# yangfei1223/CRFConv

Hardware: AMD Instinct MI355X
Metric: M points/sec fwd+bwd, S3DIS 40960-pt cloud, K=16, 3 CRF iters; mIoU parity (higher is better)
Workload: dtype f32; 1 GPU; BASELINE configs[1]: S3DIS-like synthetic clouds (one point per 4 cm voxel of an 8x8x3 m box), 4 clouds x 40960 pts per GPU, K=16, ratios [4,4,4,4,2], PointConvBig(in=6, classes=13, use_crf, steps=3), train mode: fwd + weighted CE + bwd + flat-bucket grad all-reduce + SGD(momentum) step; tables resident in HBM; point order from the device collate: morton; global_batch=4, points_per_cloud=40960, parallelism=dp1 (batch-sharded)

## Files before the change

### crfconv_amd/_lib.py

```python
import ctypes
import os

_HERE = os.path.dirname(os.path.abspath(__file__))
LIB_PATH = os.environ.get('CRFCONV_LIB') or os.path.join(_HERE, 'libcrfconv_amd.so')

_vp, _i, _i64, _sz, _f = ctypes.c_void_p, ctypes.c_int, ctypes.c_int64, ctypes.c_size_t, ctypes.c_float
_d = ctypes.c_double
_u64 = ctypes.c_uint64

SIGNATURES = {
    'crfconv_abi_version': (_i, []),
    'crfconv_last_error': (ctypes.c_char_p, []),
    'crfconv_knn': (_i, [_vp, _sz, _sz, _vp, _sz, _sz, _vp]),
    'crfconv_knn_omp': (_i, [_vp, _sz, _sz, _vp, _sz, _sz, _vp]),
    'crfconv_knn_batch': (_i, [_vp, _sz, _sz, _sz, _vp, _sz, _sz, _vp]),
    'crfconv_knn_batch_omp': (_i, [_vp, _sz, _sz, _sz, _vp, _sz, _sz, _vp]),
    'crfconv_knn_batch_dev_workspace': (_sz, [_sz, _sz, _sz, _sz]),
    'crfconv_knn_batch_dev': (_i, [_vp, _sz, _sz, _sz, _vp, _sz, _sz, _vp, _vp, _vp, _sz, _vp]),
    'crfconv_fps': (_i, [_vp, _i, _vp, _vp, _vp, _vp, _vp, _vp, _vp, _vp]),
    'crfconv_grid_subsample': (_i64, [_vp, _i64, _vp, _i, _vp, _i, _f, _vp, _vp, _vp, _i64]),
    'crfconv_grid_subsample_dev_workspace': (_sz, [_i64, _i, _i]),
    'crfconv_grid_subsample_dev': (_i64, [_vp, _i64, _vp, _i, _vp, _i, _f, _vp, _vp, _vp, _i64, _vp, _sz, _vp]),
    'crfconv_index_narrow': (_i, [_vp, _i64, _i64, _i, _i64, _vp, _vp, _vp, _vp]),
    'crfconv_index_narrow_sorted': (_i, [_vp, _i64, _i64, _i, _i64, _i, _vp, _vp, _vp, _vp]),
# ... 18 lines not shown
    'crfconv_wide_bwd_edge': (_i, [_vp, _vp, _vp, _i, _i, _i64, _i, _vp, _i, _vp]),
    'crfconv_wide_scatter': (_i, [_vp, _vp, _vp, _vp, _i, _i64, _i, _vp, _i, _vp, _vp]),
    'crfconv_wide_similarity_bwd': (_i, [_vp, _vp, _vp, _vp, _i, _i, _i64, _i, _vp, _vp, _vp]),
    'crfconv_similarity_bwd': (_i, [_vp, _vp, _vp, _vp, _i, _i, _i64, _i, _vp, _vp, _vp]),
    'crfconv_similarity_bwd_scatter': (_i, [_vp, _vp, _vp, _vp, _vp, _i, _i, _i64, _i, _vp, _vp]),
    'crfconv_pointconv_workspace': (_sz, [_i64, _i, _i]),
    'crfconv_pointconv_moments_packed': (_i, [_vp, _vp, _vp, _i, _i64, ctypes.c_double, _vp, _vp, _vp, _vp, _vp, _sz, _vp]),
    'crfconv_pointconv_moments': (_i, [_vp, _vp, _vp, _i, _i64, _vp, _vp, _sz, _vp]),
    'crfconv_pointconv_stats': (_i, [_vp, _vp, _vp, _i, _i64, _i, _vp, _vp, _vp, _f, _vp, _vp, _vp, _vp, _sz, _vp]),
    'crfconv_pointconv_forward_uv': (_i, [_vp, _vp, _vp, _vp, _i, _i64, _i, _vp, _vp, _vp, _f, _vp, _vp, _vp, _vp, _vp, _vp, _sz, _vp, _vp]),
    'crfconv_pointconv_forward_uv_hosts': (_i, [_i, _i]),
    'crfconv_pointconv_forward_uv_hosting': (_i, [_vp, _vp, _vp, _vp, _i, _i64, _i, _vp, _vp, _vp, _f, _vp, _vp, _vp, _vp, _vp, _vp, _sz, _vp,
                                                  _vp, _vp, _i, _vp, _vp, _vp]),
    'crfconv_pointconv_combine': (_i, [_vp, _vp, _vp, _vp, _vp, _vp, _d, _vp, _vp, _f, _f, _i64, _i, _vp, _vp, _vp, _vp, _vp]),
    'crfconv_pointconv_bwd_reduce_uv': (_i, [_vp, _vp, _vp, _i64, _i, _vp, _vp, _vp, _d, _i, _vp, _vp, _vp, _vp, _vp, _vp, _sz, _vp, _vp]),
    'crfconv_pointconv_forward': (_i, [_vp, _vp, _vp, _vp, _i, _i64, _i, _vp, _vp, _vp, _f, _vp, _vp, _vp, _vp]),
    'crfconv_pointconv_bwd_reduce': (_i, [_vp, _vp, _vp, _vp, _vp, _i, _i64, _i, _vp, _vp, _vp, _f, _vp, _vp, _vp, _sz, _vp]),
    'crfconv_pointconv_bwd_params': (_i, [_vp, _vp, _vp, _vp, _vp, _i, _i64, _i, _vp, _vp, _vp, _f, _vp, _vp, _vp,
                                          _vp, _vp, _vp, _sz, _vp]),
    'crfconv_pointconv_bwd_dump': (_i, [_vp, _vp, _vp, _vp, _vp, _i, _i64, _i, _vp, _vp, _vp, _f, _vp, _vp, _vp, _vp, _vp, _vp, _vp]),
    'crfconv_pointconv_bwd_a1_workspace': (_sz, [_i64, _i]),
    'crfconv_pointconv_bwd_a1': (_i, [_vp, _vp, _vp, _i64, _i, _f, _vp, _vp, _sz, _vp]),
    'crfconv_pointconv_bwd_input': (_i, [_vp, _vp, _vp, _vp, _vp, _i, _i64, _i, _vp, _vp, _vp, _f, _vp, _vp, _vp, _vp]),
    'crfconv_pointconv_bwd_input_reduce': (_i, [_vp, _vp, _vp, _vp, _vp, _i, _i64, _i64, _i, _vp, _vp, _vp, _f, _vp, _vp, _vp, _vp, _vp, _vp, _vp, _vp, _d, _i,
                                                _vp, _vp, _vp, _vp, _vp, _vp, _sz, _vp, _vp]),
    'crfconv_pointconv_fold1': (_i, [_vp, _vp, _vp, _vp, ctypes.c_double, _vp, _vp, _f, _f, _i, _i, _vp, _vp, _vp, _vp]),
    'crfconv_pointconv_fold1_batched': (_i, [_vp, _i, _vp]),
    'crfconv_pointconv_fold1_bwd_batched': (_i, [_vp, _i, _vp]),
    'crfconv_pointconv_fold1_bwd': (_i, [_vp, _vp, _vp, _vp, _vp, _f, _i, _i, _vp, _vp, _vp, _vp, _vp, _vp]),
    'crfconv_pointconv_fold2': (_i, [_vp, _vp, _vp, _vp, ctypes.c_double, _vp, _vp, _f, _f, _i, _i, _vp, _vp, _vp, _vp]),
    'crfconv_pointconv_fold2_bwd': (_i, [_vp, _vp, _vp, _vp, ctypes.c_double, _i, _i, _vp, _vp, _vp, _vp, _vp, _vp]),
    'crfconv_linear_wgrad_workspace': (_sz, [_i64, _i, _i]),
    'crfconv_linear_wgrad': (_i, [_vp, _vp, _i64, _i, _i, _vp, _vp, _vp, _sz, _vp]),
    'crfconv_random_subsets': (_i, [_vp, _vp, _vp, _vp, _i, _u64, _vp, _vp]),
    'crfconv_upindex_workspace': (_sz, [_i64, _i64]),
    'crfconv_upindex_from_table': (_i, [_vp, _vp, _vp, _vp, _i64, _i64, _i, _i64, _vp, _vp, _sz, _vp]),
    'crfconv_gather_rows_batched': (_i, [_vp, _vp, _vp, _i, _vp, _i, _i64, _i64, _i64, _vp]),
    'crfconv_argsort_codes_workspace': (_sz, [_i64, _i64]),
    'crfconv_argsort_codes': (_i, [_vp, _i64, _i64, _vp, _vp, _sz, _vp]),
    'crfconv_gridsync_workspace': (_sz, []),
    'crfconv_gridsync_fail_word': (_i, []),
    'crfconv_mlp_small_supported': (_i, [_i64, _i, _i]),
    'crfconv_mlp_small_workspace': (_sz, [_i64, _i]),
    'crfconv_mlp_small_forward': (_i, [_vp, _vp, _i64, _i, _i, _vp, _vp, _vp, _vp, _f, _f, _f, _vp, _vp, _vp, _vp, _sz, _vp, _sz, _vp]),
    'crfconv_mlp_small_forward_join': (_i, [_vp, _vp, _i64, _i, _i, _vp, _vp, _vp, _vp, _f, _f, _f, _vp, _f, _vp, _vp, _vp, _vp, _sz, _vp, _sz, _vp]),
    'crfconv_ticket_bytes': (_sz, []),
    'crfconv_mlp_backward_supported': (_i, [_i64, _i, _i]),
    'crfconv_mlp_backward_workspace': (_sz, [_i64, _i, _i]),
    'crfconv_mlp_backward': (_i, [_vp, _vp, _vp, _vp, _vp, _f, _i64, _i, _i, _vp, _vp, _vp, _vp, _vp, _sz, _vp, _vp]),
    'crfconv_linear_forward_cat': (_i, [_vp, _vp, _i, _vp, _vp, _i64, _i, _i, _vp, _vp, _vp]),
    'crfconv_linear_forward_uv_supported': (_i, [_i, _i]),
    'crfconv_linear_forward_uv': (_i, [_vp, _vp, _i64, _i, _i, _vp, _vp, _vp]),
    'crfconv_mlp_small_forward_uv_supported': (_i, [_i]),
    'crfconv_mlp_small_forward_join_uv': (_i, [_vp, _vp, _i64, _i, _i, _vp, _vp, _vp, _vp, _f, _f, _f, _vp, _f, _vp, _vp, _vp, _vp, _sz, _vp, _sz, _vp]),
    'crfconv_gemm_stats_uv_supported': (_i, [_i64, _i, _i]),
    'crfconv_gemm_stats_uv': (_i, [_vp, _vp, _i64, _i, _i, _vp, _vp, _vp]),
    'crfconv_mlp_dw_jobs': (_i, [_vp, _i, _vp]),
    'crfconv_mlp_dw_jobs_hosting': (_i, [_vp, _i, _vp, _vp, _vp, _vp, _vp, _i, _vp, _vp]),
    'crfconv_mlp_backward_add': (_i, [_vp, _vp, _vp, _vp, _vp, _f, _i64, _i, _i, _vp, _vp, _vp, _vp, _vp, _vp, _sz, _vp, _vp]),
    'crfconv_mlp_backward_add_mask': (_i, [_vp, _vp, _vp, _vp, _vp, _f, _i64, _i, _i, _vp, _f, _vp, _vp, _vp, _vp, _vp, _sz, _vp, _vp]),
    'crfconv_mlp_backward_cat': (_i, [_vp, _vp, _vp, _vp, _i, _vp, _vp, _f, _i64, _i, _i, _vp, _vp, _vp, _vp, _vp, _vp, _sz, _vp, _vp]),
    'crfconv_bn_workspace': (_sz, [_i64, _i]),
    'crfconv_bn_forward': (_i, [_vp, _i64, _i, _vp, _vp, _vp, _vp, _f, _f, _i, _f, _vp, _vp, _vp, _sz, _vp]),
    'crfconv_bn_backward': (_i, [_vp, _vp, _vp, _i64, _i, _i, _f, _vp, _vp, _vp, _vp, _sz, _vp]),
    'crfconv_bn_apply': (_i, [_vp, _i64, _i, _vp, _f, _vp, _vp]),
    'crfconv_pointconv_bwd_params_slabs': (_i, [_vp, _i64, _i, _vp, _vp, _vp]),
    'crfconv_pointconv_bwd_a1_nblk': (_i64, [_i64, _i]),
    'crfconv_reduce_jobs_f64': (_i, [_vp, _i, _vp]),
    'crfconv_pointconv_bwd_dump_jobs': (_i, [_vp, _i, _vp]),
    'crfconv_pointconv_bwd_a1_jobs': (_i, [_vp, _i, _vp]),
    'crfconv_pointconv_wide_params_supported': (_i, [_i64, _i, _i]),
    'crfconv_pointconv_wide_params_nblk': (_i64, [_i64, _i]),
    'crfconv_pointconv_wide_params_jobs': (_i, [_vp, _i, _vp]),
    'crfconv_gemm_jobs': (_i, [_vp, _i, _vp]),
    'crfconv_linear_wgrad_nblk': (_i, [_i64, _i, _i]),
    'crfconv_linear_wgrad_partial_jobs': (_i, [_vp, _i, _vp]),
    'crfconv_linear_wgrad_partial': (_i, [_vp, _vp, _i64, _i, _i, _i, _vp, _sz, _vp, _vp]),
    'crfconv_morton_codes': (_i, [_vp, _i64, _i64, _vp, _vp, _vp]),
    'crfconv_copy_jobs': (_i, [_vp, _i, _vp]),
    'crfconv_index_narrow_batched': (_i, [_vp, _i, _vp]),
    'crfconv_pointconv_moments_batched_workspace': (_sz, [_vp, _i]),
    'crfconv_pointconv_moments_batched': (_i, [_vp, _i, _vp, _sz, _vp]),
    'crfconv_reduce_jobs_both': (_i, [_vp, _i, _vp, _i, _vp]),
    'crfconv_reduce_jobs': (_i, [_vp, _i, _vp]),
    'crfconv_linear_forward_supported': (_i, [_i, _i]),
    'crfconv_linear_forward_stat_records': (_sz, [_i64]),
# ... 111 lines not shown
    _fields_ = [('x', ctypes.c_void_p), ('gout', ctypes.c_void_p), ('pos_src', ctypes.c_void_p), ('pos_tgt', ctypes.c_void_p),
                ('idx32', ctypes.c_void_p), ('K', ctypes.c_int32), ('m_tgt', ctypes.c_int64), ('d', ctypes.c_int32), ('A1', ctypes.c_void_p),
                ('b1', ctypes.c_void_p), ('W2', ctypes.c_void_p), ('slope', ctypes.c_float), ('ca', ctypes.c_void_p), ('cb', ctypes.c_void_p),
                ('cc', ctypes.c_void_p), ('dw2_partial', ctypes.c_void_p), ('a1_partial', ctypes.c_void_p)]


class PcA1Job(ctypes.Structure):
    _fields_ = [('gw', ctypes.c_void_p), ('h1', ctypes.c_void_p), ('rel', ctypes.c_void_p), ('n_edges', ctypes.c_int64), ('d', ctypes.c_int32),
                ('slope', ctypes.c_float), ('workspace', ctypes.c_void_p), ('workspace_bytes', ctypes.c_size_t)]


class GemmJob(ctypes.Structure):
    _fields_ = [('A', ctypes.c_void_p), ('B', ctypes.c_void_p), ('C', ctypes.c_void_p), ('M', ctypes.c_int64), ('N', ctypes.c_int32),
                ('K', ctypes.c_int32)]


class GemmStatsJob(ctypes.Structure):
    _fields_ = [('A', ctypes.c_void_p), ('B', ctypes.c_void_p), ('M', ctypes.c_int64), ('N', ctypes.c_int32), ('K', ctypes.c_int32),
                ('C', ctypes.c_void_p), ('stat_rec', ctypes.c_void_p)]


class BnApplyJob(ctypes.Structure):
    _fields_ = [('stat_rec', ctypes.c_void_p), ('nrec', ctypes.c_int64), ('x', ctypes.c_void_p), ('M', ctypes.c_int64), ('C', ctypes.c_int32),
                ('gamma', ctypes.c_void_p), ('beta', ctypes.c_void_p), ('run_mean', ctypes.c_void_p), ('run_var', ctypes.c_void_p),
                ('momentum', ctypes.c_float), ('eps', ctypes.c_float), ('skip', ctypes.c_void_p), ('slope', ctypes.c_float),
                ('coef', ctypes.c_void_p), ('y', ctypes.c_void_p)]


class MlpBwdJob(ctypes.Structure):
    _fields_ = [('gA', ctypes.c_void_p), ('Y', ctypes.c_void_p), ('coef', ctypes.c_void_p), ('W', ctypes.c_void_p), ('addend', ctypes.c_void_p),
                ('M', ctypes.c_int64), ('Ci', ctypes.c_int32), ('Co', ctypes.c_int32), ('training', ctypes.c_int32), ('slope', ctypes.c_float),
                ('gY', ctypes.c_void_p), ('dX', ctypes.c_void_p), ('dgamma', ctypes.c_void_p), ('dbeta', ctypes.c_void_p),
                ('workspace', ctypes.c_void_p), ('workspace_bytes', ctypes.c_size_t),
                ('mask_ref', ctypes.c_void_p), ('mask_slope', ctypes.c_float)]


class UvFold(ctypes.Structure):
    _fields_ = [('U', ctypes.c_void_p), ('V', ctypes.c_void_p), ('stats', ctypes.c_void_p), ('shift', ctypes.c_void_p),
                ('gamma2', ctypes.c_void_p), ('beta2', ctypes.c_void_p), ('n_edges', ctypes.c_double), ('run_mean', ctypes.c_void_p),
                ('run_var', ctypes.c_void_p), ('momentum', ctypes.c_float), ('eps', ctypes.c_float), ('a2', ctypes.c_void_p),
                ('b2', ctypes.c_void_p), ('aux2', ctypes.c_void_p), ('out', ctypes.c_void_p)]


class Reduce64Job(ctypes.Structure):
    _fields_ = [('partial', ctypes.c_void_p), ('is_float', ctypes.c_int32), ('nblk', ctypes.c_int64), ('nslots', ctypes.c_int32),
                ('out', ctypes.c_void_p)]


class WgradJob(ctypes.Structure):
    _fields_ = [('G', ctypes.c_void_p), ('X', ctypes.c_void_p), ('M', ctypes.c_int64), ('Co', ctypes.c_int32), ('Ci', ctypes.c_int32),
                ('want_bias', ctypes.c_int32), ('workspace', ctypes.c_void_p), ('workspace_bytes', ctypes.c_size_t)]


class RevJob(ctypes.Structure):
    _fields_ = [('idx32', ctypes.c_void_p), ('E', ctypes.c_int64), ('m_src', ctypes.c_int64), ('rev_ptr', ctypes.c_void_p),
                ('rev_eid', ctypes.c_void_p)]


class NarrowJob(ctypes.Structure):
    _fields_ = [('idx64', ctypes.c_void_p), ('B', ctypes.c_int64), ('n_tgt', ctypes.c_int64), ('K', ctypes.c_int32),
                ('n_src', ctypes.c_int64), ('sort_from', ctypes.c_int32), ('idx32', ctypes.c_void_p), ('idx16', ctypes.c_void_p),
                ('bad_count', ctypes.c_void_p)]


class MomentsJob(ctypes.Structure):
    _fields_ = [('pos_src', ctypes.c_void_p), ('pos_tgt', ctypes.c_void_p), ('idx32', ctypes.c_void_p), ('K', ctypes.c_int32),
                ('m_tgt', ctypes.c_int64), ('n_edges', ctypes.c_double), ('mean', ctypes.c_void_p), ('cov', ctypes.c_void_p),
                ('packed', ctypes.c_void_p), ('mean32', ctypes.c_void_p)]


class Fold1Job(ctypes.Structure):
    _fields_ = [('W1', ctypes.c_void_p), ('gamma1', ctypes.c_void_p), ('beta1', ctypes.c_void_p), ('mom', ctypes.c_void_p),
                ('n_edges', ctypes.c_double), ('run_mean', ctypes.c_void_p), ('run_var', ctypes.c_void_p),
                ('momentum', ctypes.c_float), ('eps', ctypes.c_float), ('use_batch', ctypes.c_int32), ('d', ctypes.c_int32),
                ('A1', ctypes.c_void_p), ('b1', ctypes.c_void_p), ('aux1', ctypes.c_void_p)]


class Fold1BwdJob(ctypes.Structure):
    _fields_ = [('W1', ctypes.c_void_p), ('gamma1', ctypes.c_void_p), ('mom', ctypes.c_void_p), ('aux1', ctypes.c_void_p),
                ('dA1b1', ctypes.c_void_p), ('eps', ctypes.c_float), ('use_batch', ctypes.c_int32), ('d', ctypes.c_int32),
                ('pad_', ctypes.c_int32), ('dW1', ctypes.c_void_p), ('dgamma1', ctypes.c_void_p), ('dbeta1', ctypes.c_void_p),
                ('dW2_f64', ctypes.c_void_p), ('dW2_f32', ctypes.c_void_p)]


# ... 47 lines not shown
```

### crfconv_amd/csrc/gemm.hip

```cpp
#include "common.hpp"
#include "gridsync.hpp"
#include "uv_fold.hpp"

#include <cstdlib>

namespace crf {

using gf32x4 = __attribute__((ext_vector_type(4))) float;

#ifndef GM_BK_
#define GM_BK_ 32
#endif
#ifndef GM_PF_
#define GM_PF_ 2
#endif
#ifndef GM_WAIT_SLEEP_
#define GM_WAIT_SLEEP_ 4
#endif
constexpr int GM_BLOCK = 256, GM_BK = GM_BK_;
constexpr int GM_PF = GM_PF_;
static_assert(GM_PF >= 2 && GM_PF % 2 == 0, "an even number of register sets (the LDS buffers alternate)");

template <bool VEC>
__device__ __forceinline__ float4 gm_ld4(const float* __restrict__ p, int valid) {
    float4 v = make_float4(0.f, 0.f, 0.f, 0.f);
    if constexpr (VEC) {
        if (valid > 0) v = *reinterpret_cast<const float4*>(p);
    } else {
        if (valid > 0) v.x = p[0];
        if (valid > 1) v.y = p[1];
        if (valid > 2) v.z = p[2];
        if (valid > 3) v.w = p[3];
    }
    return v;
}

constexpr int GM_PRO_MAXK = 512;
struct GemmPro {
    const float* Y;
    const float* coef;
    const float* fin;
    float slope;
    float* gY;
    unsigned* sync = nullptr;
    unsigned need = 0, nprod = 0;
    unsigned* fail = nullptr;
    const float* mref = nullptr;
    float mslope = 1.f;
};
constexpr int GM_PRO_LDS = 6 * GM_PRO_MAXK + 4;

template <int WM, int WN, int WR, int WC, bool BNK, bool PRO>
constexpr int gemm_lds_floats() {
    constexpr int BM = 16 * WM * WR, BN = 16 * WN * WC;
    return (PRO ? GM_PRO_LDS : 0) + 2 * BM * (GM_BK + 4) + 2 * (BNK ? BN * (GM_BK + 4) : GM_BK * (BN + 4));
}

constexpr int GM_UV_MAXK = 128;
template <int WM, int WN, int WR, int WC, bool BNK, bool VEC, bool PRO, bool STATS, bool UV = false>
__device__ __forceinline__ void gemm_tile(const float* __restrict__ A, const float* __restrict__ B,
                                          const float* __restrict__ bias, const float* __restrict__ addend,
                                          int M, int N, int K, float* __restrict__ C, const GemmPro& pro,
                                          float* __restrict__ stat_rec, const unsigned bx, const unsigned by,
                                          float* __restrict__ lds ,
                                          const unsigned gridx = 0 ,
                                          const UvFold* __restrict__ uv = nullptr, float* __restrict__ uvc = nullptr) {
    static_assert(WR * WC * WAVE == GM_BLOCK, "four wavefronts");
    static_assert(!UV || (VEC && !PRO), "the combine prologue: aligned widths, not the dX product");
    static_assert(!PRO || (VEC && !BNK), "the prologue form is the dX product of aligned widths");
    constexpr int BM = 16 * WM * WR, BN = 16 * WN * WC;
    constexpr int LDA = GM_BK + 4;
    constexpr int LDN = GM_BK + 4;
    constexpr int LDK = BN + 4;
    constexpr int TA = BM * LDA, TB = BNK ? BN * LDN : GM_BK * LDK;
    constexpr int NA4 = BM * GM_BK / 4, NB4 = BN * GM_BK / 4;
    constexpr int PA = (NA4 + GM_BLOCK - 1) / GM_BLOCK, PB = (NB4 + GM_BLOCK - 1) / GM_BLOCK;
    float* const sPro = lds;
    float (*sA)[TA] = reinterpret_cast<float (*)[TA]>(lds + (PRO ? GM_PRO_LDS : 0));
    float (*sB)[TB] = reinterpret_cast<float (*)[TB]>(lds + (PRO ? GM_PRO_LDS : 0) + 2 * TA);
    const int lane = threadIdx.x & 63, wave = threadIdx.x >> 6;
    const int rr = lane & 15, g = lane >> 4;
    const int wr = wave / WC, wc = wave - wr * WC;
    const int m0 = bx * BM, n0 = by * BN;
    const float4 zero4 = make_float4(0.f, 0.f, 0.f, 0.f);

    struct Regs { float4 a[PA], b[PB], y[(PRO || UV) ? PA : 1]; int kc; };
    auto fetch = [&](int kc, Regs& r) {
        r.kc = kc;
#pragma unroll
        for (int i = 0; i < PA; ++i) {
            const int q = threadIdx.x + GM_BLOCK * i;
            r.a[i] = zero4;
            if constexpr (PRO || UV) r.y[i] = zero4;
            if (NA4 % GM_BLOCK != 0 && q >= NA4) continue;
            const int row = m0 + q / (GM_BK / 4), k = kc + 4 * (q % (GM_BK / 4));
            if (row < M) r.a[i] = gm_ld4<VEC>(A + (int64_t)row * K + k, K - k);
            if constexpr (PRO) {
                if (row < M) r.y[i] = gm_ld4<VEC>(pro.Y + (int64_t)row * K + k, K - k);
            }
            if constexpr (UV) {
                if (row < M) r.y[i] = gm_ld4<VEC>(uv->V + (int64_t)row * K + k, K - k);
            }
        }
#pragma unroll
        for (int i = 0; i < PB; ++i) {
            const int q = threadIdx.x + GM_BLOCK * i;
            r.b[i] = zero4;
            if (NB4 % GM_BLOCK != 0 && q >= NB4) continue;
            if constexpr (BNK) {
                const int n = n0 + q / (GM_BK / 4), k = kc + 4 * (q % (GM_BK / 4));
                if (n < N) r.b[i] = gm_ld4<VEC>(B + (int64_t)n * K + k, K - k);
            } else {
                const int k = kc + q / (BN / 4), n = n0 + 4 * (q % (BN / 4));
                if (k < K) r.b[i] = gm_ld4<VEC>(B + (int64_t)k * N + n, N - n);
            }
        }
    };
    auto park = [&](int buf, const Regs& r) {
#pragma unroll
        for (int i = 0; i < PA; ++i) {
            const int q = threadIdx.x + GM_BLOCK * i;
            if (NA4 % GM_BLOCK != 0 && q >= NA4) continue;
            float4 av = r.a[i];
            if constexpr (PRO) {
                const int row = m0 + q / (GM_BK / 4), k = r.kc + 4 * (q % (GM_BK / 4));
                if (row < M && k < K) {
                    const float4 ca = *reinterpret_cast<const float4*>(sPro + k), cb = *reinterpret_cast<const float4*>(sPro + GM_PRO_MAXK + k);
                    const float4 mu = *reinterpret_cast<const float4*>(sPro + 2 * GM_PRO_MAXK + k), rs = *reinterpret_cast<const float4*>(sPro + 3 * GM_PRO_MAXK + k);
                    const float4 c2 = *reinterpret_cast<const float4*>(sPro + 4 * GM_PRO_MAXK + k), c3 = *reinterpret_cast<const float4*>(sPro + 5 * GM_PRO_MAXK + k);
// ... 160 lines not shown
                    s2[e] += __shfl_xor(s2[e], o, WAVE);
                }
            }
            if (rr == 0 && n < N) {
#pragma unroll
                for (int e = 0; e < 4; ++e)
                    *reinterpret_cast<float4*>(stat_rec + ((int64_t)rec * N + n + e) * 4) = make_float4(sv[e], (float)nrows, s1[e], s2[e]);
            }
        }
    }
#pragma unroll
    for (int i = 0; i < WM; ++i) {
        const int row = m0 + 16 * (wr * WM + i) + rr;
        if (row >= M) continue;
#pragma unroll
        for (int j = 0; j < WN; ++j) {
            const int n = n0 + 16 * (wc * WN + j) + 4 * g;
            if (n >= N) continue;
            float4 o = make_float4(acc[i][j][0], acc[i][j][1], acc[i][j][2], acc[i][j][3]);
            if (addend != nullptr) {
                const float4 a4 = gm_ld4<VEC>(addend + (int64_t)row * N + n, N - n);
                o.x += a4.x; o.y += a4.y; o.z += a4.z; o.w += a4.w;
            }
            if constexpr (PRO) {
                if (pro.mref != nullptr) {
                    const float4 r4 = gm_ld4<VEC>(pro.mref + (int64_t)row * N + n, N - n);
                    o.x = r4.x > 0.f ? o.x : pro.mslope * o.x;
                    o.y = r4.y > 0.f ? o.y : pro.mslope * o.y;
                    o.z = r4.z > 0.f ? o.z : pro.mslope * o.z;
                    o.w = r4.w > 0.f ? o.w : pro.mslope * o.w;
                }
            }
            float* cp = C + (int64_t)row * N + n;
            if constexpr (VEC) {
                *reinterpret_cast<float4*>(cp) = o;
            } else {
                cp[0] = o.x;
                if (n + 1 < N) cp[1] = o.y;
                if (n + 2 < N) cp[2] = o.z;
                if (n + 3 < N) cp[3] = o.w;
            }
        }
    }
    if constexpr (PRO) {
        if (pro.sync != nullptr && threadIdx.x == 0) {
            const unsigned local = bx + by * gridx, g = local % (unsigned)WL_GROUPS;
            const unsigned n_in_group = pro.nprod / WL_GROUPS + (g < pro.nprod % WL_GROUPS ? 1u : 0u);
            unsigned* gt = pro.sync + (WL_REPL + g) * FW_LINE;
            if (__hip_atomic_fetch_add(gt, 1u, __ATOMIC_RELAXED, __HIP_MEMORY_SCOPE_AGENT) + 1 == n_in_group) {
                __hip_atomic_store(gt, 0u, __ATOMIC_RELAXED, __HIP_MEMORY_SCOPE_AGENT);
                unsigned* top = pro.sync + (WL_REPL + WL_GROUPS) * FW_LINE;
                const unsigned groups = pro.nprod < (unsigned)WL_GROUPS ? pro.nprod : (unsigned)WL_GROUPS;
                if (__hip_atomic_fetch_add(top, 1u, __ATOMIC_RELAXED, __HIP_MEMORY_SCOPE_AGENT) + 1 == groups) {
                    __hip_atomic_store(top, 0u, __ATOMIC_RELAXED, __HIP_MEMORY_SCOPE_AGENT);
                    for (int r = 0; r < WL_REPL; ++r) __hip_atomic_store(pro.sync + r * FW_LINE, 0u, __ATOMIC_RELAXED, __HIP_MEMORY_SCOPE_AGENT);
                }
            }
        }
    }
}

template <int WM, int WN, int WR, int WC, bool BNK, bool VEC, bool PRO = false, bool STATS = false>
__global__ __launch_bounds__(GM_BLOCK) void gemm_kernel(const float* __restrict__ A, const float* __restrict__ B,
                                                        const float* __restrict__ bias, const float* __restrict__ addend,
                                                        int M, int N, int K, float* __restrict__ C, const GemmPro pro = GemmPro(),
                                                        float* __restrict__ stat_rec = nullptr) {
// ... 27 lines not shown
static inline bool gm_wide(int64_t M, int N) { return N >= GM_WIDE_MIN_N_ && ((M + 31) / 32) * (int64_t)((N + 31) / 32) >= GM_WIDE_MIN_TILES_; }
struct GemmStatsJobs {
    const float* A[GG_MAX]; const float* B[GG_MAX]; float* C[GG_MAX]; float* rec[GG_MAX];
    int M[GG_MAX], N[GG_MAX], K[GG_MAX], tiles_x[GG_MAX], wide[GG_MAX];
    int tile_base[GG_MAX + 1];
    int njobs;
};
__global__ __launch_bounds__(GM_BLOCK) void gemm_stats_jobs_kernel(const GemmStatsJobs t) {
    int j = 0;
    while (j + 1 < t.njobs && t.tile_base[j + 1] <= (int)blockIdx.x) ++j;
    const unsigned local = blockIdx.x - (unsigned)t.tile_base[j];
    const unsigned tx = (unsigned)uni(t.tiles_x[j]);
    const unsigned bx = (unsigned)uni((int)(local % tx)), by = (unsigned)uni((int)(local / tx));
    __shared__ __attribute__((aligned(16))) float lds[gemm_lds_floats<1, 2, 2, 2, true, false>()];
    if (uni(t.wide[j]))
        gemm_tile<1, 2, 2, 2, true, true, false, true>(uni(t.A[j]), uni(t.B[j]), nullptr, nullptr, uni(t.M[j]), uni(t.N[j]), uni(t.K[j]), uni(t.C[j]), GemmPro(),
                                                       uni(t.rec[j]), bx, by, lds);
    else
        gemm_tile<1, 1, 2, 2, true, true, false, true>(uni(t.A[j]), uni(t.B[j]), nullptr, nullptr, uni(t.M[j]), uni(t.N[j]), uni(t.K[j]), uni(t.C[j]), GemmPro(),
                                                       uni(t.rec[j]), bx, by, lds);
}
__global__ __launch_bounds__(GM_BLOCK) void gemm_stats_uv_kernel(const float* __restrict__ U, const float* __restrict__ B, const int M, const int N,
                                                                 const int K, float* __restrict__ C, float* __restrict__ rec, const int tiles_x,
                                                                 const int wide, const UvFold uv) {
    const unsigned tx = (unsigned)tiles_x;
    const unsigned bx = (unsigned)uni((int)(blockIdx.x % tx)), by = (unsigned)uni((int)(blockIdx.x / tx));
    __shared__ __attribute__((aligned(16))) float lds[gemm_lds_floats<1, 2, 2, 2, true, false>()];
    __shared__ __attribute__((aligned(16))) float s_uv[2 * GM_UV_MAXK];
    if (wide)
        gemm_tile<1, 2, 2, 2, true, true, false, true, true>(U, B, nullptr, nullptr, M, N, K, C, GemmPro(), rec, bx, by, lds, 0, &uv, s_uv);
    else
        gemm_tile<1, 1, 2, 2, true, true, false, true, true>(U, B, nullptr, nullptr, M, N, K, C, GemmPro(), rec, bx, by, lds, 0, &uv, s_uv);
}
struct GemmProJobs {
    const float* A[GG_MAX]; const float* B[GG_MAX]; const float* addend[GG_MAX]; float* C[GG_MAX];
    GemmPro pro[GG_MAX];
    int M[GG_MAX], N[GG_MAX], K[GG_MAX], tiles_x[GG_MAX], wide[GG_MAX];
    int tile_base[GG_MAX + 1];
    int njobs;
};
__global__ __launch_bounds__(GM_BLOCK) void gemm_pro_jobs_kernel(const GemmProJobs t) {
    int j = 0;
    while (j + 1 < t.njobs && t.tile_base[j + 1] <= (int)blockIdx.x) ++j;
    const unsigned local = blockIdx.x - (unsigned)t.tile_base[j];
    GemmPro pro;
    pro.Y = uni(t.pro[j].Y); pro.coef = uni(t.pro[j].coef); pro.fin = uni(t.pro[j].fin); pro.slope = uni(t.pro[j].slope); pro.gY = uni(t.pro[j].gY);
    pro.mref = uni(t.pro[j].mref); pro.mslope = uni(t.pro[j].mslope);
    const unsigned tx = (unsigned)uni(t.tiles_x[j]);
    const unsigned bx = (unsigned)uni((int)(local % tx)), by = (unsigned)uni((int)(local / tx));
    __shared__ __attribute__((aligned(16))) float lds[gemm_lds_floats<1, 2, 2, 2, false, true>()];
    if (uni(t.wide[j]))
        gemm_tile<1, 2, 2, 2, false, true, true, false>(uni(t.A[j]), uni(t.B[j]), nullptr, uni(t.addend[j]), uni(t.M[j]), uni(t.N[j]), uni(t.K[j]), uni(t.C[j]),
                                                        pro, nullptr, bx, by, lds, tx);
    else
        gemm_tile<1, 1, 2, 2, false, true, true, false>(uni(t.A[j]), uni(t.B[j]), nullptr, uni(t.addend[j]), uni(t.M[j]), uni(t.N[j]), uni(t.K[j]), uni(t.C[j]),
                                                        pro, nullptr, bx, by, lds, tx);
}

}

namespace crf {

constexpr int BT_ROWS = 128, BT_CH = 64, BT_NR = BT_ROWS / 16;
struct TileSumFin {
    unsigned* ticket;
    int ntile;
    int training;
    float inv_m;
    float* fin;
    float* dgamma;
    float* dbeta;
    unsigned* done = nullptr;
};
struct TileSumLds { float red[16][2][64]; int last; };
typedef unsigned int bt_u32x2 __attribute__((ext_vector_type(2)));
__device__ __forceinline__ void bn_bwd_tile_sums_body(const float* __restrict__ gA, const float* __restrict__ Y,
                                                       const float* __restrict__ coef, int M, int K, int tile_rows,
                                                       float slope, double* __restrict__ partial, const int bx, const int by,
                                                       const TileSumFin f, TileSumLds& L) {
    float (&s_red)[16][2][64] = L.red;
    int& s_last = L.last;
    const int cq = threadIdx.x & 15, rl = threadIdx.x >> 4;
    const int c = by * BT_CH + 4 * cq;
    const int row0 = bx * tile_rows;
    const int row_end = row0 + tile_rows < M ? row0 + tile_rows : M;
    float4 s1 = make_float4(0.f, 0.f, 0.f, 0.f), s2 = s1;
    if (c < K) {
        const float4 ca = *reinterpret_cast<const float4*>(coef + c), cb = *reinterpret_cast<const float4*>(coef + K + c);
// ... 70 lines not shown
        if (threadIdx.x < WL_REPL) __hip_atomic_fetch_add(f.done + threadIdx.x * FW_LINE, 1u, __ATOMIC_RELAXED, __HIP_MEMORY_SCOPE_AGENT);
    }
}

struct TileSumJobs {
    const float* gA[GG_MAX]; const float* Y[GG_MAX]; const float* coef[GG_MAX]; double* partial[GG_MAX];
    float* fin[GG_MAX]; float* dgamma[GG_MAX]; float* dbeta[GG_MAX];
    int M[GG_MAX], K[GG_MAX], tile_rows[GG_MAX], ntile[GG_MAX], training[GG_MAX];
    float slope[GG_MAX], inv_m[GG_MAX];
    unsigned* ticket;
    int blk_base[GG_MAX + 1];
    int njobs;
};
constexpr int BT_SLABS = GM_PRO_MAXK / BT_CH;
__device__ __forceinline__ void bn_bwd_tile_sums_job(const TileSumJobs& t, const int blk, TileSumLds& L, unsigned* const* done = nullptr) {
    int j = 0;
    while (j + 1 < t.njobs && t.blk_base[j + 1] <= blk) ++j;
    const int local = blk - t.blk_base[j];
    const int ntile = uni(t.ntile[j]);
    const int bx = local % ntile, by = local / ntile;
    TileSumFin f;
    f.ticket = uni(t.ticket) + (j * BT_SLABS + by) * FW_LINE; f.ntile = ntile; f.training = uni(t.training[j]); f.inv_m = uni(t.inv_m[j]);
    f.fin = uni(t.fin[j]); f.dgamma = uni(t.dgamma[j]); f.dbeta = uni(t.dbeta[j]);
    f.done = done != nullptr ? uni(done[j]) : nullptr;
    bn_bwd_tile_sums_body(uni(t.gA[j]), uni(t.Y[j]), uni(t.coef[j]), uni(t.M[j]), uni(t.K[j]), uni(t.tile_rows[j]), uni(t.slope[j]), uni(t.partial[j]),
                          bx, by, f, L);
}
__global__ __launch_bounds__(256) void bn_bwd_tile_sums_jobs_kernel(const TileSumJobs t) {
    __shared__ TileSumLds L;
    bn_bwd_tile_sums_job(t, (int)blockIdx.x, L);
}

struct SmallBwdSync { unsigned* done[GG_MAX]; int nsum; };
__global__ __launch_bounds__(GM_BLOCK) void mlp_small_bwd_jobs_kernel(const TileSumJobs ts, const GemmProJobs t, const SmallBwdSync sy) {
    __shared__ __attribute__((aligned(16))) float lds[gemm_lds_floats<1, 2, 2, 2, false, true>()];
    static_assert(sizeof(TileSumLds) <= sizeof(lds), "the tile-sum workgroups use the product's buffer");
    if ((int)blockIdx.x < sy.nsum) {
        bn_bwd_tile_sums_job(ts, (int)blockIdx.x, *reinterpret_cast<TileSumLds*>(lds), sy.done);
        return;
    }
    const int blk = (int)blockIdx.x - sy.nsum;
    int j = 0;
    while (j + 1 < t.njobs && t.tile_base[j + 1] <= blk) ++j;
    const unsigned local = (unsigned)(blk - t.tile_base[j]);
    GemmPro pro;
    pro.Y = uni(t.pro[j].Y); pro.coef = uni(t.pro[j].coef); pro.fin = uni(t.pro[j].fin); pro.slope = uni(t.pro[j].slope); pro.gY = uni(t.pro[j].gY);
    pro.mref = uni(t.pro[j].mref); pro.mslope = uni(t.pro[j].mslope);
    pro.sync = uni(t.pro[j].sync); pro.need = (unsigned)uni((int)t.pro[j].need); pro.nprod = (unsigned)uni((int)t.pro[j].nprod); pro.fail = uni(t.pro[j].fail);
    const unsigned tx = (unsigned)uni(t.tiles_x[j]);
    const unsigned bx = (unsigned)uni((int)(local % tx)), by = (unsigned)uni((int)(local / tx));
    if (uni(t.wide[j]))
        gemm_tile<1, 2, 2, 2, false, true, true, false>(uni(t.A[j]), uni(t.B[j]), nullptr, uni(t.addend[j]), uni(t.M[j]), uni(t.N[j]), uni(t.K[j]), uni(t.C[j]),
                                                        pro, nullptr, bx, by, lds, tx);
    else
        gemm_tile<1, 1, 2, 2, false, true, true, false>(uni(t.A[j]), uni(t.B[j]), nullptr, uni(t.addend[j]), uni(t.M[j]), uni(t.N[j]), uni(t.K[j]), uni(t.C[j]),
                                                        pro, nullptr, bx, by, lds, tx);
}
}

extern "C" int crfconv_mlp_small_backward_supported(int64_t M, int Ci, int Co) {
    return (M >= 1 && M < (int64_t)1 << 24 && Ci >= 4 && Co >= 4 && Ci % 4 == 0 && Co % 4 == 0 && Co <= crf::GM_PRO_MAXK) ? 1 : 0;
}

static void bt_plan(int64_t M, int& ntile, int& tile_rows) {
    constexpr int BT_MAXTILES = 48;
    int64_t rows = crf::BT_ROWS;
    if ((M + rows - 1) / rows > BT_MAXTILES) rows = (((M + BT_MAXTILES - 1) / BT_MAXTILES + 15) / 16) * 16;
    tile_rows = (int)rows;
    ntile = (int)((M + rows - 1) / rows);
}

static size_t bt_fin_offset(int Co, int ntile) { return (sizeof(double) * 2 * (size_t)Co * (size_t)ntile + 255) & ~(size_t)255; }
extern "C" size_t crfconv_mlp_small_backward_workspace(int64_t M, int Co) {
    if (M < 1 || Co < 1) return 0;
    int ntile, tile_rows;
    bt_plan(M, ntile, tile_rows);
    return bt_fin_offset(Co, ntile) + sizeof(float) * 2 * (size_t)Co + 512;
}

extern "C" int crfconv_mlp_small_backward(const float* gA, const float* Y, const float* coef, const float* W, const float* addend,
                                          int64_t M, int Ci, int Co, int training, float slope, float* gY, float* dX, float* dgamma,
                                          float* dbeta, void* workspace, size_t workspace_bytes, unsigned* ticket, void* stream) {
    crf_mlp_bwd_job job;
    job.gA = gA; job.Y = Y; job.coef = coef; job.W = W; job.addend = addend; job.M = M; job.Ci = Ci; job.Co = Co; job.training = training;
    job.slope = slope; job.gY = gY; job.dX = dX; job.dgamma = dgamma; job.dbeta = dbeta; job.workspace = workspace; job.workspace_bytes = workspace_bytes;
    job.mask_ref = nullptr; job.mask_slope = 1.f;
    return crfconv_mlp_small_backward_jobs(&job, 1, ticket, stream);
}

static int mlp_small_backward_jobs_impl(const crf_mlp_bwd_job* jobs, int njobs, unsigned* ticket, unsigned* sync_ws, void* stream);
extern "C" int crfconv_mlp_small_backward_jobs(const crf_mlp_bwd_job* jobs, int njobs, unsigned* ticket, void* stream) {
    return mlp_small_backward_jobs_impl(jobs, njobs, ticket, nullptr, stream);
}
extern "C" int crfconv_mlp_small_backward_jobs_one_launch(const crf_mlp_bwd_job* jobs, int njobs, unsigned* ticket, unsigned* sync_ws, void* stream) {
    CRF_REQUIRE(sync_ws != nullptr, CRF_ERR_ARG, "null barrier workspace");
    return mlp_small_backward_jobs_impl(jobs, njobs, ticket, sync_ws, stream);
}
static int mlp_small_backward_jobs_impl(const crf_mlp_bwd_job* jobs, int njobs, unsigned* ticket, unsigned* sync_ws, void* stream) {
    CRF_REQUIRE(jobs && ticket && njobs >= 1 && njobs <= crf::GG_MAX, CRF_ERR_ARG, "1 .. %d jobs (got %d) and the ticket words", crf::GG_MAX, njobs);
    crf::TileSumJobs ts;
    crf::GemmProJobs gp;
    crf::SmallBwdSync sy;
    for (int j = 0; j < crf::GG_MAX; ++j) sy.done[j] = nullptr;
    sy.nsum = 0;
    int64_t blocks = 0, tiles = 0;
    for (int j = 0; j <= crf::GG_MAX; ++j) {
        ts.blk_base[j] = (int)blocks;
        gp.tile_base[j] = (int)tiles;
        if (j >= crf::GG_MAX) break;
        if (j >= njobs) {
            ts.gA[j] = nullptr; ts.Y[j] = nullptr; ts.coef[j] = nullptr; ts.partial[j] = nullptr; ts.M[j] = 0; ts.K[j] = 4; ts.tile_rows[j] = crf::BT_ROWS;
            ts.ntile[j] = 1; ts.slope[j] = 1.f; ts.fin[j] = nullptr; ts.dgamma[j] = nullptr; ts.dbeta[j] = nullptr; ts.training[j] = 0; ts.inv_m[j] = 0.f;
            gp.A[j] = nullptr; gp.B[j] = nullptr; gp.addend[j] = nullptr; gp.C[j] = nullptr; gp.pro[j] = crf::GemmPro(); gp.M[j] = 0; gp.N[j] = 4; gp.K[j] = 4;
            gp.tiles_x[j] = 1; gp.wide[j] = 0;
            continue;
        }
        const crf_mlp_bwd_job& b = jobs[j];
        CRF_REQUIRE(b.gA && b.Y && b.coef && b.W && b.gY && b.dX && b.dgamma && b.dbeta && b.workspace, CRF_ERR_ARG, "job %d: null pointer", j);
        CRF_REQUIRE(crfconv_mlp_small_backward_supported(b.M, b.Ci, b.Co), CRF_ERR_UNSUPPORTED,
                    "job %d: mlp_small_backward %lld x %d -> %d: widths must be multiples of 4, Co <= %d", j, (long long)b.M, b.Ci, b.Co, crf::GM_PRO_MAXK);
        CRF_REQUIRE(b.workspace_bytes >= crfconv_mlp_small_backward_workspace(b.M, b.Co), CRF_ERR_WORKSPACE, "job %d: workspace too small", j);
        double* partial = reinterpret_cast<double*>((reinterpret_cast<uintptr_t>(b.workspace) + 255) & ~(uintptr_t)255);
        int ntile, tile_rows;
        bt_plan(b.M, ntile, tile_rows);
        ts.gA[j] = b.gA; ts.Y[j] = b.Y; ts.coef[j] = b.coef; ts.partial[j] = partial; ts.M[j] = (int)b.M; ts.K[j] = b.Co; ts.tile_rows[j] = tile_rows;
        float* fin = reinterpret_cast<float*>(reinterpret_cast<char*>(partial) + bt_fin_offset(b.Co, ntile));
        ts.ntile[j] = ntile; ts.slope[j] = b.slope; ts.fin[j] = fin; ts.dgamma[j] = b.dgamma; ts.dbeta[j] = b.dbeta; ts.training[j] = b.training;
        ts.inv_m[j] = (float)(1.0 / (double)b.M);
        blocks += (int64_t)ntile * ((b.Co + crf::BT_CH - 1) / crf::BT_CH);
        crf::GemmPro pro;
        pro.Y = b.Y; pro.coef = b.coef; pro.fin = fin; pro.slope = b.slope; pro.gY = b.gY;
        pro.mref = b.mask_ref; pro.mslope = b.mask_slope;
        gp.A[j] = b.gA; gp.B[j] = b.W; gp.addend[j] = b.addend; gp.C[j] = b.dX; gp.pro[j] = pro; gp.M[j] = (int)b.M; gp.N[j] = b.Ci; gp.K[j] = b.Co;
        gp.tiles_x[j] = (int)((b.M + 31) / 32);
        gp.wide[j] = crf::gm_wide(b.M, b.Ci) ? 1 : 0;
        const int64_t jt = (int64_t)gp.tiles_x[j] * ((b.Ci + (gp.wide[j] ? 63 : 31)) / (gp.wide[j] ? 64 : 32));
        tiles += jt;
        CRF_REQUIRE(tiles + blocks < ((int64_t)1 << 31), CRF_ERR_UNSUPPORTED, "too many tiles in one batch");
        if (sync_ws != nullptr) {
            gp.pro[j].sync = sync_ws + (crf::FW_WAIT + j * crf::WL_LINES) * crf::FW_LINE;
            gp.pro[j].need = (unsigned)((b.Co + crf::BT_CH - 1) / crf::BT_CH);
            gp.pro[j].nprod = (unsigned)jt;
            gp.pro[j].fail = sync_ws + crf::FW_FAIL * crf::FW_LINE;
            sy.done[j] = gp.pro[j].sync;
        }
    }
    ts.njobs = njobs;
    ts.ticket = ticket;
    gp.njobs = njobs;
    hipStream_t st = crf::as_stream(stream);
    if (sync_ws != nullptr) {
        sy.nsum = (int)blocks;
        hipLaunchKernelGGL(crf::mlp_small_bwd_jobs_kernel, dim3((unsigned)(blocks + tiles)), dim3(crf::GM_BLOCK), 0, st, ts, gp, sy);
        CRF_LAUNCH_CHECK();
        return CRF_OK;
    }
    hipLaunchKernelGGL(crf::bn_bwd_tile_sums_jobs_kernel, dim3((unsigned)blocks), dim3(256), 0, st, ts);
    CRF_LAUNCH_CHECK();
    hipLaunchKernelGGL(crf::gemm_pro_jobs_kernel, dim3((unsigned)tiles), dim3(crf::GM_BLOCK), 0, st, gp);
    CRF_LAUNCH_CHECK();
    return CRF_OK;
}

extern "C" size_t crfconv_gemm_stat_records(int64_t M) { return M < 1 ? 0 : (size_t)(2 * ((M + 31) / 32)); }

extern "C" int crfconv_gemm_stats(const float* A, const float* B, int64_t M, int N, int K, float* C, float* stat_rec, void* stream) {
    crf_gemm_stats_job job;
    job.A = A; job.B = B; job.M = M; job.N = N; job.K = K; job.C = C; job.stat_rec = stat_rec;
    return crfconv_gemm_stats_jobs(&job, 1, stream);
}

extern "C" int crfconv_gemm_stats_jobs(const crf_gemm_stats_job* jobs, int njobs, void* stream) {
    CRF_REQUIRE(jobs && njobs >= 1 && njobs <= crf::GG_MAX, CRF_ERR_ARG, "1 .. %d jobs (got %d)", crf::GG_MAX, njobs);
    crf::GemmStatsJobs t;
    int64_t tiles = 0;
    for (int j = 0; j <= crf::GG_MAX; ++j) {
        t.tile_base[j] = (int)tiles;
        if (j >= crf::GG_MAX) break;
        if (j >= njobs) {
            t.A[j] = nullptr; t.B[j] = nullptr; t.C[j] = nullptr; t.rec[j] = nullptr; t.M[j] = 0; t.N[j] = 4; t.K[j] = 4; t.tiles_x[j] = 1; t.wide[j] = 0;
            continue;
        }
        const crf_gemm_stats_job& b = jobs[j];
        CRF_REQUIRE(b.A && b.B && b.C && b.stat_rec, CRF_ERR_ARG, "job %d: null pointer", j);
        CRF_REQUIRE(b.M >= 1 && b.M < ((int64_t)1 << 31) && b.N >= 4 && b.K >= 4 && b.N % 4 == 0 && b.K % 4 == 0, CRF_ERR_UNSUPPORTED,
                    "job %d: gemm_stats %lld x %d x %d: N and K must be multiples of 4", j, (long long)b.M, b.N, b.K);
        t.A[j] = b.A; t.B[j] = b.B; t.C[j] = b.C; t.rec[j] = b.stat_rec; t.M[j] = (int)b.M; t.N[j] = b.N; t.K[j] = b.K;
        t.tiles_x[j] = (int)((b.M + 31) / 32);
        t.wide[j] = crf::gm_wide(b.M, b.N) ? 1 : 0;
        tiles += (int64_t)t.tiles_x[j] * ((b.N + (t.wide[j] ? 63 : 31)) / (t.wide[j] ? 64 : 32));
        CRF_REQUIRE(tiles < ((int64_t)1 << 31), CRF_ERR_UNSUPPORTED, "too many tiles in one batch");
    }
    t.njobs = njobs;
    hipLaunchKernelGGL(crf::gemm_stats_jobs_kernel, dim3((unsigned)tiles), dim3(crf::GM_BLOCK), 0, crf::as_stream(stream), t);
    CRF_LAUNCH_CHECK();
    return CRF_OK;
}

extern "C" int crfconv_gemm_stats_uv_supported(int64_t M, int N, int K) {
    return (M >= 1 && M < ((int64_t)1 << 31) && N >= 4 && K >= 4 && N % 4 == 0 && K % 4 == 0 && K <= crf::GM_UV_MAXK) ? 1 : 0;
}
extern "C" int crfconv_gemm_stats_uv(const crf_uv_fold* f, const float* B, int64_t M, int N, int K, float* C, float* stat_rec, void* stream) {
    CRF_REQUIRE(B && C && stat_rec, CRF_ERR_ARG, "null pointer");
    CRF_REQUIRE(crf::uv_fold_complete(f), CRF_ERR_ARG, "combine record: null pointer, or running statistics not as a pair");
    CRF_REQUIRE(crfconv_gemm_stats_uv_supported(M, N, K), CRF_ERR_UNSUPPORTED, "gemm_stats_uv %lld x %d x %d: N, K multiples of 4, K <= %d",
                (long long)M, N, K, crf::GM_UV_MAXK);
    const crf::UvFold uv = crf::uv_fold_args(f);
    const int tiles_x = (int)((M + 31) / 32), wide = crf::gm_wide(M, N) ? 1 : 0;
    const int64_t tiles = (int64_t)tiles_x * ((N + (wide ? 63 : 31)) / (wide ? 64 : 32));
    CRF_REQUIRE(tiles < ((int64_t)1 << 31), CRF_ERR_UNSUPPORTED, "too many tiles");
    hipLaunchKernelGGL(crf::gemm_stats_uv_kernel, dim3((unsigned)tiles), dim3(crf::GM_BLOCK), 0, crf::as_stream(stream), f->U, B, (int)M, N, K, C,
                       stat_rec, tiles_x, wide, uv);
    CRF_LAUNCH_CHECK();
    return CRF_OK;
}

extern "C" int crfconv_gemm_jobs(const crf_gemm_job* jobs, int njobs, void* stream) {
    CRF_REQUIRE(jobs || njobs == 0, CRF_ERR_ARG, "null pointer");
    CRF_REQUIRE(njobs >= 0, CRF_ERR_ARG, "njobs=%d < 0", njobs);
    hipStream_t st = crf::as_stream(stream);
    for (int j0 = 0; j0 < njobs; j0 += crf::GJ_MAX) {
        crf::GemmJobs t;
        const int n = njobs - j0 < crf::GJ_MAX ? njobs - j0 : crf::GJ_MAX;
        int64_t tiles = 0;
        for (int j = 0; j <= crf::GJ_MAX; ++j) {
            t.tile_base[j] = (int)tiles;
            if (j < n) {
                const crf_gemm_job& jb = jobs[j0 + j];
                CRF_REQUIRE(jb.A && jb.B && jb.C, CRF_ERR_ARG, "job %d: null pointer", j0 + j);
                CRF_REQUIRE(jb.M >= 1 && jb.M < ((int64_t)1 << 31) && jb.N >= 4 && jb.K >= 4 && jb.N % 4 == 0 && jb.K % 4 == 0, CRF_ERR_UNSUPPORTED,
                            "job %d: %lld x %d x %d (N, K multiples of 4)", j0 + j, (long long)jb.M, jb.N, jb.K);
                t.A[j] = jb.A; t.B[j] = jb.B; t.C[j] = jb.C; t.M[j] = (int)jb.M; t.N[j] = jb.N; t.K[j] = jb.K;
                t.tiles_x[j] = (int)((jb.M + 31) / 32);
                tiles += (int64_t)t.tiles_x[j] * ((jb.N + 31) / 32);
                CRF_REQUIRE(tiles < ((int64_t)1 << 31), CRF_ERR_UNSUPPORTED, "too many tiles in one batch");
            } else if (j < crf::GJ_MAX) {
                t.A[j] = nullptr; t.B[j] = nullptr; t.C[j] = nullptr; t.M[j] = 0; t.N[j] = 4; t.K[j] = 4; t.tiles_x[j] = 1;
            }
        }
        t.njobs = n;
        hipLaunchKernelGGL(crf::gemm_jobs_kernel, dim3((unsigned)tiles), dim3(crf::GM_BLOCK), 0, st, t);
        CRF_LAUNCH_CHECK();
    }
    return CRF_OK;
}
// ... 38 lines not shown
```

### crfconv_amd/csrc/linear.hip

```cpp
#include "common.hpp"
#include "gridsync.hpp"
#include "wgrad_body.hpp"
#include "crf_matrices_body.hpp"
#include "reduce64_body.hpp"
#include "uv_fold.hpp"

#include <cstdlib>

namespace crf {

template <int TCO, int TCI>
__global__ __launch_bounds__(WG_BLOCK) void wgrad_kernel(const float* __restrict__ G,
                                                         const float* __restrict__ X, int64_t M, int Co,
                                                         int Ci, int rows_per_block,
                                                         float* __restrict__ partial ,
                                                         float* __restrict__ partial_b ) {
    __shared__ float s_red[WG_RED_BUFS * TCO * TCI * 256];
    __shared__ float s_b[WG_WAVES * TCO * 16];
    wgrad_body<TCO, TCI>(G, X, M, Co, Ci, rows_per_block, partial, partial_b, blockIdx.x, blockIdx.y, blockIdx.z, s_red, s_b);
}

__global__ __launch_bounds__(WG_BLOCK) void wgrad_jobs_any_kernel(const WgJobTable t) {
    __shared__ float s_red[WG_RED_BUFS * 4 * 4 * 256];
    __shared__ float s_b[WG_WAVES * 4 * 16];
    wgrad_any_run(t, (int)blockIdx.x, s_red, s_b);
}


__device__ __forceinline__ void mlp_channel_part(int c, double s1, double s2, const float* __restrict__ coef, int64_t M, int Co,
                                                 float* __restrict__ dgamma, float* __restrict__ dbeta, float* __restrict__ bcoef) {
    dbeta[c] = (float)s1;
    dgamma[c] = (float)s2;
    const double a = coef[c], mu = coef[2 * Co + c], rs = coef[3 * Co + c];
    const double c2 = s1 / (double)M, c3 = s2 / (double)M;
    bcoef[c] = coef[c];
    bcoef[Co + c] = coef[Co + c];
    bcoef[2 * Co + c] = (float)a;
    bcoef[3 * Co + c] = (float)(-a * c3 * rs);
    bcoef[4 * Co + c] = (float)(-a * c2 + a * c3 * rs * mu);
}

template <int TCO, int TCI>
__global__ __launch_bounds__(WG_BLOCK) void mlp_bwd_p1_kernel(const float* __restrict__ GA, const float* __restrict__ Y,
                                                              const float* __restrict__ X,
                                                              const float* __restrict__ X2, int split ,
                                                              const float* __restrict__ coef ,
                                                              float slope, int64_t M, int Co, int Ci, int rows_per_block,
                                                              float* __restrict__ PA ,
                                                              float* __restrict__ PB ,
                                                              float* __restrict__ PG ,
                                                              float* __restrict__ PX ,
                                                              unsigned* __restrict__ ticket ,
// ... 350 lines not shown
    CRF_LAUNCH_CHECK();
    return CRF_OK;
}

extern "C" int crfconv_linear_wgrad_partial(const float* G, const float* X, int64_t M, int Co, int Ci, int want_bias,
                                            void* workspace, size_t workspace_bytes, int* nblk_out, crf_stream_t stream) {
    CRF_REQUIRE(G && X && workspace && nblk_out, CRF_ERR_ARG, "null pointer");
    CRF_REQUIRE(M > 0 && Co > 0 && Ci > 0 && Co <= 4096 && Ci <= 4096, CRF_ERR_ARG, "bad shape M=%lld Co=%d Ci=%d",
                (long long)M, Co, Ci);
    CRF_REQUIRE((reinterpret_cast<uintptr_t>(workspace) & 255) == 0, CRF_ERR_ARG, "workspace must be 256-byte aligned");
    CRF_REQUIRE(workspace_bytes >= crfconv_linear_wgrad_workspace(M, Co, Ci), CRF_ERR_WORKSPACE, "workspace too small");
    const WgPlan p = wg_plan(M, Co, Ci);
    float* partial = reinterpret_cast<float*>(workspace);
    float* partial_b = want_bias ? partial + (size_t)p.nblk * Co * Ci : nullptr;
    *nblk_out = p.nblk;
    return wgrad_launch(G, X, M, Co, Ci, p, partial, partial_b, as_stream(stream));
}

extern "C" int crfconv_linear_wgrad_nblk(int64_t M, int Co, int Ci) {
    if (M <= 0 || Co <= 0 || Ci <= 0) return 0;
    return wg_plan(M, Co, Ci).nblk;
}

extern "C" int crfconv_linear_wgrad_partial_jobs(const crf_wgrad_job* jobs, int njobs, crf_stream_t stream) {
    CRF_REQUIRE(jobs || njobs == 0, CRF_ERR_ARG, "null pointer");
    CRF_REQUIRE(njobs >= 0, CRF_ERR_ARG, "njobs=%d < 0", njobs);
    hipStream_t st = as_stream(stream);
    for (int j = 0; j < njobs; ++j) {
        const crf_wgrad_job& jb = jobs[j];
        CRF_REQUIRE(jb.G && jb.X && jb.workspace, CRF_ERR_ARG, "job %d: null pointer", j);
        CRF_REQUIRE(jb.M > 0 && jb.M < ((int64_t)1 << 31) && jb.Co > 0 && jb.Ci > 0 && jb.Co <= 4096 && jb.Ci <= 4096, CRF_ERR_ARG,
                    "job %d: bad shape M=%lld Co=%d Ci=%d", j, (long long)jb.M, jb.Co, jb.Ci);
        CRF_REQUIRE((reinterpret_cast<uintptr_t>(jb.workspace) & 255) == 0, CRF_ERR_ARG, "job %d: workspace must be 256-byte aligned", j);
        CRF_REQUIRE(jb.workspace_bytes >= crfconv_linear_wgrad_workspace(jb.M, jb.Co, jb.Ci), CRF_ERR_WORKSPACE, "job %d: workspace too small", j);
    }
    for (int j0 = 0; j0 < njobs; j0 += WJ_MAX) {
        WgJobTable t;
        int64_t blocks = 0;
        const int n = njobs - j0 < WJ_MAX ? njobs - j0 : WJ_MAX;
        wg_fill_table(jobs + j0, n, t, blocks);
        CRF_REQUIRE(blocks < ((int64_t)1 << 31), CRF_ERR_UNSUPPORTED, "too many workgroups in one batch");
        hipLaunchKernelGGL(wgrad_jobs_any_kernel, dim3((unsigned)blocks), dim3(WG_BLOCK), 0, st, t);
        CRF_LAUNCH_CHECK();
    }
    return CRF_OK;
}

extern "C" int crfconv_reduce_jobs(const crf_reduce_job* jobs, int njobs, crf_stream_t stream) {
    CRF_REQUIRE(jobs || njobs == 0, CRF_ERR_ARG, "null pointer");
    CRF_REQUIRE(njobs >= 0, CRF_ERR_ARG, "njobs=%d < 0", njobs);
    hipStream_t st = as_stream(stream);
    for (int j0 = 0; j0 < njobs; j0 += RJ_MAX) {
        ReduceJobTable tbl;
        const int n = njobs - j0 < RJ_MAX ? njobs - j0 : RJ_MAX;
        int64_t total = 0;
        for (int j = 0; j < n; ++j) {
            const crf_reduce_job& jb = jobs[j0 + j];
            CRF_REQUIRE(jb.partial && jb.out && jb.nblk > 0 && jb.nslots > 0, CRF_ERR_ARG, "job %d is malformed", j0 + j);
            tbl.partial[j] = jb.partial;
            tbl.out[j] = jb.out;
            tbl.nblk[j] = jb.nblk;
            tbl.nslots[j] = jb.nslots;
            tbl.group_begin[j] = (int)total;
            total += (jb.nslots + 63) / 64;
            CRF_REQUIRE(total < ((int64_t)1 << 30), CRF_ERR_ARG, "too many slots in one batch");
        }
        for (int j = n; j <= RJ_MAX; ++j) tbl.group_begin[j] = (int)total;
// ... 36 lines not shown
            t.partial[j] = jb.partial; t.out[j] = jb.out; t.is_float[j] = jb.is_float; t.nblk[j] = (int)jb.nblk; t.nslots[j] = jb.nslots;
            waves += jb.nslots;
        } else if (j < R64_MAX) {
            t.partial[j] = nullptr; t.out[j] = nullptr; t.is_float[j] = 0; t.nblk[j] = 0; t.nslots[j] = 0;
        }
    }
    t.njobs = njobs64;
    const int64_t n64 = cdiv(waves, 256 / WAVE);
    CRF_REQUIRE(total + n64 < ((int64_t)1 << 30), CRF_ERR_UNSUPPORTED, "too many slots in one batch");
    hipLaunchKernelGGL(reduce_both_kernel, dim3((unsigned)(total + n64)), dim3(256), 0, as_stream(stream), tbl, t, (int)n64);
    CRF_LAUNCH_CHECK();
    return CRF_OK;
}

extern "C" int crfconv_linear_wgrad(const float* G, const float* X, int64_t M, int Co, int Ci, float* dW,
                                    float* db, void* workspace, size_t workspace_bytes, crf_stream_t stream) {
    CRF_REQUIRE(G && X && dW && workspace, CRF_ERR_ARG, "null pointer");
    CRF_REQUIRE(M > 0 && Co > 0 && Ci > 0 && Co <= 4096 && Ci <= 4096, CRF_ERR_ARG, "bad shape M=%lld Co=%d Ci=%d",
                (long long)M, Co, Ci);
    CRF_REQUIRE(workspace_bytes >= crfconv_linear_wgrad_workspace(M, Co, Ci), CRF_ERR_WORKSPACE, "workspace too small");
    const WgPlan p = wg_plan(M, Co, Ci);
    hipStream_t st = as_stream(stream);
    float* partial = reinterpret_cast<float*>((reinterpret_cast<uintptr_t>(workspace) + 255) & ~(uintptr_t)255);
    float* partial_b = db ? partial + (size_t)p.nblk * Co * Ci : nullptr;
    if (int rc = wgrad_launch(G, X, M, Co, Ci, p, partial, partial_b, st)) return rc;
    hipLaunchKernelGGL(wgrad_reduce_kernel, dim3((unsigned)cdiv((int64_t)Co * Ci, 64)), dim3(256), 0, st, partial, p.nblk,
                       Co * Ci, dW);
    CRF_LAUNCH_CHECK();
    if (db) {
        hipLaunchKernelGGL(wgrad_reduce_kernel, dim3((unsigned)cdiv((int64_t)Co, 64)), dim3(256), 0, st, partial_b, p.nblk,
                           Co, db);
        CRF_LAUNCH_CHECK();
    }
    return CRF_OK;
}

namespace crf {
__device__ __forceinline__ void gauss_jordan_tiles(double (&t)[4][4], int H, double (*s_row)[64], double (*s_col)[64]) {
    const int tr = threadIdx.x >> 4, tc = threadIdx.x & 15;
#pragma unroll
    for (int ip = 0; ip < 4; ++ip) {
        for (int pp = 0; pp < 16; ++pp) {
            const int p = 16 * ip + pp;
            if (p >= H) break;
            const int b = p & 1;
            if (tr == pp) {
#pragma unroll
                for (int j = 0; j < 4; ++j) s_row[b][tc + 16 * j] = t[ip][j];
            }
            if (tc == pp) {
#pragma unroll
                for (int i = 0; i < 4; ++i) s_col[b][tr + 16 * i] = t[i][ip];
            }
            __syncthreads();
            const double piv = 1.0 / s_row[b][p];
            double rowv[4], colv[4];
#pragma unroll
            for (int j = 0; j < 4; ++j) rowv[j] = s_row[b][tc + 16 * j] * piv;
#pragma unroll
            for (int i = 0; i < 4; ++i) colv[i] = s_col[b][tr + 16 * i];
#pragma unroll
            for (int i = 0; i < 4; ++i)
#pragma unroll
                for (int j = 0; j < 4; ++j) {
                    const bool rp = (i == ip) && (tr == pp), cp = (j == ip) && (tc == pp);
                    const double upd = t[i][j] - colv[i] * rowv[j];
// ... 1183 lines not shown
```

### crfconv_amd/csrc/mlp_small.hip

```cpp
#include "common.hpp"
#include "gridsync.hpp"
#include "uv_fold.hpp"

namespace crf {

using f32x4s = __attribute__((ext_vector_type(4))) float;

constexpr int SM_BLOCK = 256, SM_ROWS = 64, SM_COLS = 64, SM_KC = 64, SM_LD = SM_KC + 4;
#ifndef SM_MAX_ROWS_
#define SM_MAX_ROWS_ 4096
#endif
constexpr int64_t SM_MAX_ROWS = SM_MAX_ROWS_;
#ifndef SM_MIN_BLOCKS
#define SM_MIN_BLOCKS 256
#endif

constexpr int SM_UV_MAXK = 128;
template <int TCO, bool UV>
__device__ __forceinline__ void mlp_small_fwd_body(const float* __restrict__ X, const float* __restrict__ W,
                                                   int M, int Ci, int Co, const float* __restrict__ gamma,
                                                   const float* __restrict__ beta, float* __restrict__ run_mean,
                                                   float* __restrict__ run_var, float momentum, float eps,
                                                   float slope, float* __restrict__ Y, float* __restrict__ A,
                                                   float* __restrict__ coef, float* __restrict__ rec,
                                                   unsigned* __restrict__ sync_ws,
                                                   const float* __restrict__ skip, float join_slope, const UvFold& uv) {
    __shared__ float sWbuf[2][SM_COLS * SM_LD];
    __shared__ __attribute__((aligned(16))) float s_uv[UV ? 2 : 1][UV ? SM_UV_MAXK : 4];
    __shared__ double s_comb[2][SM_BLOCK];
    __shared__ float s_ab[2][SM_COLS];
    __shared__ int s_ok;
    float* const sW = sWbuf[0];
    const int lane = threadIdx.x & 63, wave = threadIdx.x >> 6;
    const int rr = lane & 15, g = lane >> 4;
    constexpr int COLS = 16 * TCO;
    const int rb = blockIdx.x, co_base = blockIdx.y * COLS;
    const int r = rb * SM_ROWS + wave * 16 + rr;
    const bool rv = r < M;
    const float* xrow = X + (int64_t)(rv ? r : 0) * Ci;
    const float4 zero4 = make_float4(0.f, 0.f, 0.f, 0.f);
    [[maybe_unused]] const float* vrow = UV ? uv.V + (int64_t)(rv ? r : 0) * Ci : nullptr;
    if constexpr (UV) {
        if ((int)threadIdx.x < Ci) {
            const int c = threadIdx.x;
            const UvCoef k = uv_coef(c, Ci, uv.stats, uv.shift, uv.gamma, uv.beta, uv.n_edges, uv.eps);
            s_uv[0][c] = k.a;
            s_uv[1][c] = uv_vcoef(k);
            if (blockIdx.x == 0 && blockIdx.y == 0)
                uv_publish(c, Ci, k, uv.n_edges, uv.run_mean, uv.run_var, uv.momentum, uv.a2, uv.b2, uv.aux2);
        }
    }
    [[maybe_unused]] auto form = [&](int k0, float4 u, float4 v) -> float4 {
        if (!(rv && k0 < Ci)) return zero4;
        const float4 o = uv_out4(ld4(&s_uv[0][k0]), ld4(&s_uv[1][k0]), u, v);
        if (blockIdx.y == 0) st4(uv.out + (int64_t)r * Ci + k0, o);
        return o;
    };

    f32x4s acc[TCO];
#pragma unroll
    for (int t = 0; t < TCO; ++t) acc[t] = f32x4s{0.f, 0.f, 0.f, 0.f};

    const int wr = threadIdx.x >> 4, k4 = threadIdx.x & 15;
    const float* wsrc = W + (int64_t)(co_base + wr) * Ci + 4 * k4;
    float4 wreg[TCO], xv[4], xn[4];
    [[maybe_unused]] float4 vn[UV ? 4 : 1];
#pragma unroll
    for (int i = 0; i < TCO; ++i) wreg[i] = 4 * k4 < Ci ? ld4(wsrc + (int64_t)16 * i * Ci) : zero4;
#pragma unroll
    for (int c = 0; c < 4; ++c) {
        const int k0 = 16 * c + 4 * g;
        xv[c] = (rv && k0 < Ci) ? ld4(xrow + k0) : zero4;
        if constexpr (UV) vn[c] = (rv && k0 < Ci) ? ld4(vrow + k0) : zero4;
    }
#pragma unroll
    for (int i = 0; i < TCO; ++i) st4(sWbuf[0] + (wr + 16 * i) * SM_LD + 4 * k4, wreg[i]);
    __syncthreads();
    if constexpr (UV) {
#pragma unroll
        for (int c = 0; c < 4; ++c) xv[c] = form(16 * c + 4 * g, xv[c], vn[c]);
    }
    int cur = 0;
    for (int kc = 0; kc < Ci; kc += SM_KC) {
        const int kn = kc + SM_KC;
        const bool more = kn < Ci;
        if (more) {
#pragma unroll
            for (int i = 0; i < TCO; ++i) wreg[i] = kn + 4 * k4 < Ci ? ld4(wsrc + (int64_t)16 * i * Ci + kn) : zero4;
#pragma unroll
            for (int c = 0; c < 4; ++c) {
                const int k0 = kn + 16 * c + 4 * g;
                xn[c] = (rv && k0 < Ci) ? ld4(xrow + k0) : zero4;
                if constexpr (UV) vn[c] = (rv && k0 < Ci) ? ld4(vrow + k0) : zero4;
            }
        }
        const float* sWc = sWbuf[cur];
#pragma unroll
        for (int c = 0; c < 4; ++c) {
#pragma unroll
            for (int t = 0; t < TCO; ++t) {
                const float4 wv = ld4(sWc + (16 * t + rr) * SM_LD + 16 * c + 4 * g);
                acc[t] = __builtin_amdgcn_mfma_f32_16x16x4f32(wv.x, xv[c].x, acc[t], 0, 0, 0);
                acc[t] = __builtin_amdgcn_mfma_f32_16x16x4f32(wv.y, xv[c].y, acc[t], 0, 0, 0);
                acc[t] = __builtin_amdgcn_mfma_f32_16x16x4f32(wv.z, xv[c].z, acc[t], 0, 0, 0);
                acc[t] = __builtin_amdgcn_mfma_f32_16x16x4f32(wv.w, xv[c].w, acc[t], 0, 0, 0);
            }
        }
        if (more) {
#pragma unroll
            for (int i = 0; i < TCO; ++i) st4(sWbuf[cur ^ 1] + (wr + 16 * i) * SM_LD + 4 * k4, wreg[i]);
#pragma unroll
            for (int c = 0; c < 4; ++c) {
                if constexpr (UV) xv[c] = form(kn + 16 * c + 4 * g, xn[c], vn[c]);
                else xv[c] = xn[c];
            }
        }
        __syncthreads();
        cur ^= 1;
    }
    if (rv) {
#pragma unroll
        for (int t = 0; t < TCO; ++t)
            st4(Y + (int64_t)r * Co + co_base + 16 * t + 4 * g, make_float4(acc[t][0], acc[t][1], acc[t][2], acc[t][3]));
    }

// ... 120 lines not shown
                o.z = o.z > 0.f ? o.z : o.z * join_slope; o.w = o.w > 0.f ? o.w : o.w * join_slope;
            }
            st4(A + (int64_t)r * Co + co_base + 16 * t + 4 * g, o);
        }
    }
    fused_exit_reset(sync_ws, nblk, 2, bid);
}

template <int TCO>
__global__ __launch_bounds__(SM_BLOCK) void mlp_small_fwd_kernel(const float* __restrict__ X, const float* __restrict__ W,
                                                                 int M, int Ci, int Co, const float* __restrict__ gamma,
                                                                 const float* __restrict__ beta, float* __restrict__ run_mean,
                                                                 float* __restrict__ run_var, float momentum, float eps,
                                                                 float slope, float* __restrict__ Y, float* __restrict__ A,
                                                                 float* __restrict__ coef, float* __restrict__ rec,
                                                                 unsigned* __restrict__ sync_ws,
                                                                 const float* __restrict__ skip, float join_slope) {
    mlp_small_fwd_body<TCO, false>(X, W, M, Ci, Co, gamma, beta, run_mean, run_var, momentum, eps, slope, Y, A, coef, rec, sync_ws, skip,
                                   join_slope, UvFold());
}
template <int TCO>
__global__ __launch_bounds__(SM_BLOCK) void mlp_small_fwd_uv_kernel(const float* __restrict__ U, const float* __restrict__ W,
                                                                    int M, int Ci, int Co, const float* __restrict__ gamma,
                                                                    const float* __restrict__ beta, float* __restrict__ run_mean,
                                                                    float* __restrict__ run_var, float momentum, float eps,
                                                                    float slope, float* __restrict__ Y, float* __restrict__ A,
                                                                    float* __restrict__ coef, float* __restrict__ rec,
                                                                    unsigned* __restrict__ sync_ws,
                                                                    const float* __restrict__ skip, float join_slope, const UvFold uv) {
    mlp_small_fwd_body<TCO, true>(U, W, M, Ci, Co, gamma, beta, run_mean, run_var, momentum, eps, slope, Y, A, coef, rec, sync_ws, skip,
                                  join_slope, uv);
}

static int mlp_small_capacity() {
    static int cap = -1;
    if (cap < 0) {
        int dev = 0, cus = 0, per_cu = 0;
        if (hipGetDevice(&dev) != hipSuccess) return 0;
        if (hipDeviceGetAttribute(&cus, hipDeviceAttributeMultiprocessorCount, dev) != hipSuccess) return 0;
        int per_cu_uv = 0;
        if (hipOccupancyMaxActiveBlocksPerMultiprocessor(&per_cu, mlp_small_fwd_kernel<4>, SM_BLOCK, 0) != hipSuccess) return 0;
        if (hipOccupancyMaxActiveBlocksPerMultiprocessor(&per_cu_uv, mlp_small_fwd_uv_kernel<4>, SM_BLOCK, 0) != hipSuccess) return 0;
        if (per_cu_uv < per_cu) per_cu = per_cu_uv;
        if (per_cu > 2) per_cu = 2;
        cap = cus * per_cu;
    }
    return cap;
}

static bool mlp_small_shape_ok(int64_t M, int Ci, int Co) {
    return M >= 1 && M <= SM_MAX_ROWS && Ci >= 16 && Ci % 16 == 0 && Ci <= 1024 && Co >= SM_COLS && Co % SM_COLS == 0 && Co <= 1024;
}

static int mlp_small_tco(int64_t M, int Co, int cap) {
    const int64_t rb = cdiv(M, SM_ROWS);
    for (int tco = 4; tco >= 1; tco >>= 1) {
        const int64_t nblk = rb * (Co / (16 * tco));
        if (nblk > cap) return 0;
        if (nblk >= SM_MIN_BLOCKS || tco == 1) return tco;
    }
    return 0;
}

}

using namespace crf;

extern "C" size_t crfconv_gridsync_workspace(void) { return FW_TOTAL_WORDS * sizeof(unsigned); }

extern "C" int crfconv_gridsync_fail_word(void) { return FW_FAIL * FW_LINE; }

extern "C" int crfconv_mlp_small_supported(int64_t M, int Ci, int Co) {
    if (!mlp_small_shape_ok(M, Ci, Co)) return 0;
    return mlp_small_tco(M, Co, mlp_small_capacity()) > 0 ? 1 : 0;
}

extern "C" size_t crfconv_mlp_small_workspace(int64_t M, int Co) {
    if (M < 1 || Co < 1) return 0;
    return (size_t)cdiv(M, SM_ROWS) * (size_t)Co * 4 * sizeof(float);
}

static int mlp_small_forward_impl(const float* X, const float* W, int64_t M, int Ci, int Co, const float* gamma,
                                  const float* beta, float* run_mean, float* run_var, float momentum, float eps,
                                  float slope, const float* skip, float join_slope, float* Y, float* A, float* coef, void* ws,
                                  size_t ws_bytes, void* sync_ws, size_t sync_bytes, crf_stream_t stream, const UvFold* uv = nullptr) {
    CRF_REQUIRE(X && W && gamma && beta && Y && A && coef && ws && sync_ws, CRF_ERR_ARG, "null pointer");
    CRF_REQUIRE(mlp_small_shape_ok(M, Ci, Co), CRF_ERR_UNSUPPORTED, "shape m=%lld Ci=%d Co=%d outside the one-launch kernel",
                (long long)M, Ci, Co);
    CRF_REQUIRE(ws_bytes >= crfconv_mlp_small_workspace(M, Co), CRF_ERR_WORKSPACE, "workspace too small");
    CRF_REQUIRE(sync_bytes >= crfconv_gridsync_workspace(), CRF_ERR_WORKSPACE, "barrier words: %zu bytes, need %zu", sync_bytes,
                crfconv_gridsync_workspace());
    const int tco = mlp_small_tco(M, Co, mlp_small_capacity());
    CRF_REQUIRE(tco > 0, CRF_ERR_UNSUPPORTED, "the workgroups of m=%lld Co=%d cannot all be resident (capacity %d)", (long long)M, Co,
                mlp_small_capacity());
    const dim3 grid((unsigned)cdiv(M, SM_ROWS), (unsigned)(Co / (16 * tco)));
#define SMF(T) hipLaunchKernelGGL(mlp_small_fwd_kernel<T>, grid, dim3(SM_BLOCK), 0, as_stream(stream), X, W, (int)M, Ci, Co, gamma, beta, \
                                  run_mean, run_var, momentum, eps, slope, Y, A, coef, reinterpret_cast<float*>(ws),               \
                                  reinterpret_cast<unsigned*>(sync_ws), skip, join_slope)
#define SMU(T) hipLaunchKernelGGL(mlp_small_fwd_uv_kernel<T>, grid, dim3(SM_BLOCK), 0, as_stream(stream), X, W, (int)M, Ci, Co, gamma, beta, \
                                  run_mean, run_var, momentum, eps, slope, Y, A, coef, reinterpret_cast<float*>(ws),                  \
                                  reinterpret_cast<unsigned*>(sync_ws), skip, join_slope, *uv)
    if (uv != nullptr) {
        if (tco == 4) SMU(4);
        else if (tco == 2) SMU(2);
        else SMU(1);
    } else if (tco == 4) SMF(4);
    else if (tco == 2) SMF(2);
    else SMF(1);
#undef SMU
#undef SMF
    CRF_LAUNCH_CHECK();
    return CRF_OK;
}

extern "C" int crfconv_mlp_small_forward(const float* X, const float* W, int64_t M, int Ci, int Co, const float* gamma,
                                         const float* beta, float* run_mean, float* run_var, float momentum, float eps,
                                         float slope, float* Y, float* A, float* coef, void* ws, size_t ws_bytes,
                                         void* sync_ws, size_t sync_bytes, crf_stream_t stream) {
    return mlp_small_forward_impl(X, W, M, Ci, Co, gamma, beta, run_mean, run_var, momentum, eps, slope, nullptr, 1.f, Y, A, coef, ws,
                                  ws_bytes, sync_ws, sync_bytes, stream);
}

extern "C" int crfconv_mlp_small_forward_join(const float* X, const float* W, int64_t M, int Ci, int Co, const float* gamma,
                                              const float* beta, float* run_mean, float* run_var, float momentum, float eps,
                                              float slope, const float* skip, float join_slope, float* Y, float* A, float* coef,
                                              void* ws, size_t ws_bytes, void* sync_ws, size_t sync_bytes, crf_stream_t stream) {
    CRF_REQUIRE(skip, CRF_ERR_ARG, "null pointer");
    return mlp_small_forward_impl(X, W, M, Ci, Co, gamma, beta, run_mean, run_var, momentum, eps, slope, skip, join_slope, Y, A, coef,
                                  ws, ws_bytes, sync_ws, sync_bytes, stream);
}

extern "C" int crfconv_mlp_small_forward_uv_supported(int Ci) { return (Ci >= 16 && Ci % 16 == 0 && Ci <= SM_UV_MAXK) ? 1 : 0; }

extern "C" int crfconv_mlp_small_forward_join_uv(const crf_uv_fold* f, const float* W, int64_t M, int Ci, int Co, const float* gamma,
                                                 const float* beta, float* run_mean, float* run_var, float momentum, float eps,
                                                 float slope, const float* skip, float join_slope, float* Y, float* A, float* coef,
                                                 void* ws, size_t ws_bytes, void* sync_ws, size_t sync_bytes, crf_stream_t stream) {
    CRF_REQUIRE(skip, CRF_ERR_ARG, "null pointer");
    CRF_REQUIRE(uv_fold_complete(f), CRF_ERR_ARG, "combine record: null pointer, or running statistics not as a pair");
    CRF_REQUIRE(crfconv_mlp_small_forward_uv_supported(Ci), CRF_ERR_UNSUPPORTED, "combine prologue: Ci=%d outside 16..%d", Ci, SM_UV_MAXK);
    const UvFold uv = uv_fold_args(f);
    return mlp_small_forward_impl(f->U, W, M, Ci, Co, gamma, beta, run_mean, run_var, momentum, eps, slope, skip, join_slope, Y, A, coef,
                                  ws, ws_bytes, sync_ws, sync_bytes, stream, &uv);
}
```

### crfconv_amd/csrc/wgrad_body.hpp

```cpp
#pragma once
#include "common.hpp"

namespace crf {

using f32x4 = __attribute__((ext_vector_type(4))) float;

constexpr int WG_BLOCK = 256;
constexpr int WG_WAVES = WG_BLOCK / WAVE;
#ifndef WG_RED_BUFS_
#define WG_RED_BUFS_ 2
#endif
constexpr int WG_RED_BUFS = WG_RED_BUFS_;

template <int TCO, int TCI>
__device__ __forceinline__ void wgrad_body(const float* __restrict__ G, const float* __restrict__ X, int64_t M, int Co, int Ci,
                                           int rows_per_block, float* __restrict__ partial ,
                                           float* __restrict__ partial_b , int bx, int by, int bz,
                                           float* __restrict__ s_red_ , float* __restrict__ s_b_ ) {
    const int lane = threadIdx.x & 63, wave = threadIdx.x >> 6;
    const int co_base = by * 16 * TCO, ci_base = bz * 16 * TCI;
    const int kk = lane >> 4, cc = lane & 15;
    f32x4 acc[TCO][TCI];
#pragma unroll
    for (int a = 0; a < TCO; ++a)
#pragma unroll
        for (int b = 0; b < TCI; ++b) acc[a][b] = f32x4{0.f, 0.f, 0.f, 0.f};
    float bsum[TCO];
#pragma unroll
    for (int a = 0; a < TCO; ++a) bsum[a] = 0.f;

    const int64_t row_begin = (int64_t)bx * rows_per_block;
    const int64_t row_end = row_begin + rows_per_block < M ? row_begin + rows_per_block : M;
#ifndef WG_PREFETCH_
#define WG_PREFETCH_ 0
#endif
    struct Frag { float av[4][TCO], bv[4][TCI]; };
    auto load = [&](int64_t r0, Frag& f) {
#pragma unroll
        for (int u = 0; u < 4; ++u) {
            const int64_t r = r0 + 4 * u + kk;
            const bool rv = r < row_end;
#pragma unroll
            for (int a = 0; a < TCO; ++a) {
                const int co = co_base + 16 * a + cc;
                f.av[u][a] = (rv && co < Co) ? G[r * Co + co] : 0.f;
            }
#pragma unroll
            for (int b = 0; b < TCI; ++b) {
                const int ci = ci_base + 16 * b + cc;
                f.bv[u][b] = (rv && ci < Ci) ? X[r * Ci + ci] : 0.f;
            }
// ... 33 lines not shown
#pragma unroll
        for (int a = 0; a < TCO; ++a)
#pragma unroll
            for (int b = 0; b < TCI; ++b)
#pragma unroll
                for (int g = 0; g < 4; ++g) s_red[wave % WG_RED_BUFS][(a * TCI + b) * 256 + (4 * kk + g) * 16 + cc] = acc[a][b][g];
    };
#pragma unroll
    for (int a = 0; a < TCO; ++a) {
        float t = bsum[a];
        t += __shfl_xor(t, 16, WAVE);
        t += __shfl_xor(t, 32, WAVE);
        if (kk == 0) s_b[wave][a * 16 + cc] = t;
    }
    float v[PER];
#pragma unroll
    for (int rd = 0; rd < WG_WAVES / WG_RED_BUFS; ++rd) {
        if (rd > 0) __syncthreads();
        if (wave / WG_RED_BUFS == rd) park();
        __syncthreads();
#pragma unroll
        for (int i = 0; i < PER; ++i) {
            const int t = threadIdx.x + WG_BLOCK * i;
#pragma unroll
            for (int b = 0; b < WG_RED_BUFS; ++b) v[i] = (rd == 0 && b == 0) ? s_red[0][t] : v[i] + s_red[b][t];
        }
    }
    const int64_t pb = (int64_t)bx;
#pragma unroll
    for (int i = 0; i < PER; ++i) {
        const int t = threadIdx.x + WG_BLOCK * i;
        const int tile = t >> 8, a = tile / TCI, b = tile % TCI, r = (t >> 4) & 15, j = t & 15;
        const int co = co_base + 16 * a + r, ci = ci_base + 16 * b + j;
        if (co < Co && ci < Ci) partial[(pb * Co + co) * Ci + ci] = v[i];
    }
    if (partial_b != nullptr && bz == 0) {
        for (int t = threadIdx.x; t < TCO * 16; t += WG_BLOCK) {
            float v = 0.f;
#pragma unroll
            for (int w = 0; w < WG_WAVES; ++w) v += s_b[w][t];
            const int co = co_base + t;
            if (co < Co) partial_b[pb * Co + co] = v;
        }
    }
}

constexpr int WJ_MAX = 48;
struct WgJobTable {
    const float* G[WJ_MAX];
    const float* X[WJ_MAX];
    float* partial[WJ_MAX];
    float* partial_b[WJ_MAX];
    int M[WJ_MAX], Co[WJ_MAX], Ci[WJ_MAX], rows_per_block[WJ_MAX], nblk[WJ_MAX], gy[WJ_MAX];
    int blk_base[WJ_MAX + 1];
    int njobs;
    unsigned char cls[WJ_MAX];
};
__device__ __forceinline__ void wgrad_any_run(const WgJobTable& t, int blk, float* s_red, float* s_b) {
    int lo = 0, hi = t.njobs;
    while (hi - lo > 1) {
        const int mid = (lo + hi) >> 1;
        if (t.blk_base[mid] <= blk) lo = mid; else hi = mid;
    }
    const int local = blk - t.blk_base[lo];
    const int bx = local % t.nblk[lo], rest = local / t.nblk[lo];
    const int by = rest % t.gy[lo], bz = rest / t.gy[lo];
#define WB(TA, TB) wgrad_body<TA, TB>(t.G[lo], t.X[lo], t.M[lo], t.Co[lo], t.Ci[lo], t.rows_per_block[lo], t.partial[lo], t.partial_b[lo], bx, by, bz, s_red, s_b)
    switch (t.cls[lo]) {
        case 44: WB(4, 4); break;
        case 22: WB(2, 2); break;
        case 42: WB(4, 2); break;
        case 24: WB(2, 4); break;
        case 14: WB(1, 4); break;
        case 41: WB(4, 1); break;
        case 12: WB(1, 2); break;
        case 21: WB(2, 1); break;
        default: WB(1, 1); break;
    }
#undef WB
}

struct WgPlan {
    int tco, tci, gy, gz, nblk, rows_per_block;
};
#ifndef WG_LONG_ROWS_
#define WG_LONG_ROWS_ 256
#endif


static WgPlan wg_plan(int64_t M, int Co, int Ci) {
    WgPlan p;
    const int t_co = (Co + 15) / 16, t_ci = (Ci + 15) / 16;
    p.tco = t_co >= 4 ? 4 : (t_co >= 2 ? 2 : 1);
    p.tci = t_ci >= 4 ? 4 : (t_ci >= 2 ? 2 : 1);
    p.gy = (t_co + p.tco - 1) / p.tco;
    p.gz = (t_ci + p.tci - 1) / p.tci;
    int64_t slices = 512 / ((int64_t)p.gy * p.gz);
    if (slices < 32) slices = 32;
    int64_t rows = (M + slices - 1) / slices;
    if (rows < 64) rows = 64;
    rows = (rows + 63) / 64 * 64;
#if WG_LONG_ROWS_ > 64
    if (M <= 65536) {
        int64_t want = WG_LONG_ROWS_;
        if (M < 2 * want) want = ((M + 1) / 2 + 63) / 64 * 64;
        if (rows < want) rows = want;
    }
#endif
    p.rows_per_block = (int)rows;
    p.nblk = (int)((M + rows - 1) / rows);
    return p;
}


static inline void wg_fill_table(const crf_wgrad_job* jobs, int n, WgJobTable& t, int64_t& blocks) {
    blocks = 0;
    for (int k = 0; k < n; ++k) {
        const crf_wgrad_job& jb = jobs[k];
        const WgPlan p = wg_plan(jb.M, jb.Co, jb.Ci);
        float* partial = reinterpret_cast<float*>(jb.workspace);
        t.G[k] = jb.G; t.X[k] = jb.X; t.partial[k] = partial;
        t.partial_b[k] = jb.want_bias ? partial + (size_t)p.nblk * jb.Co * jb.Ci : nullptr;
        t.M[k] = (int)jb.M; t.Co[k] = jb.Co; t.Ci[k] = jb.Ci; t.rows_per_block[k] = p.rows_per_block; t.nblk[k] = p.nblk; t.gy[k] = p.gy;
        t.cls[k] = (unsigned char)(10 * p.tco + p.tci);
        t.blk_base[k] = (int)blocks;
        blocks += (int64_t)p.nblk * p.gy * p.gz;
    }
    for (int k = n; k <= WJ_MAX; ++k) t.blk_base[k] = (int)blocks;
    for (int k = n; k < WJ_MAX; ++k) {
        t.G[k] = nullptr; t.X[k] = nullptr; t.partial[k] = nullptr; t.partial_b[k] = nullptr;
        t.M[k] = 0; t.Co[k] = 1; t.Ci[k] = 1; t.rows_per_block[k] = 64; t.nblk[k] = 1; t.gy[k] = 1; t.cls[k] = 11;
    }
    t.njobs = n;
}

}
```

### crfconv_amd/ops/_base.py

```python
import ctypes

import torch

from .. import _lib
from ..graph import NeighborTable, ptr, require_gpu, stream_ptr

BN_EPS = 1e-5


def _f32c(t):
    if t.dtype is torch.float32 and t.is_contiguous():
        return t.detach()
    return t.detach().to(torch.float32).contiguous()


def _pad_channels(t, C):
    if t.shape[-1] == C:
        return t
    return torch.nn.functional.pad(t, (0, C - t.shape[-1]))


def _next_supported(c, choices):
    for v in choices:
        if c <= v:
# ... 84 lines not shown
            if code != 0:
                ws.zero_()
                bad.append((key, code))
    remote = False
    if reduced_flag is not None and reduced_flag.numel():
        v = float(reduced_flag.reshape(-1)[0].item())
        remote = not (v == 0.0)
        if remote:
            reduced_flag.zero_()
    if bad or remote:
        state.small_mlp_disabled = True
        where = ('device(s) %s (code 0x%x)' % (sorted({k[0] for k, _ in bad}), bad[0][1])) if bad else 'another rank of the process group'
        raise _lib.CrfConvError('grid barrier timed out on %s: a one-launch kernel could not get all its '
                                'workgroups resident; its outputs were poisoned with NaN.  The one-launch MLP path is now '
                                'disabled for this process (CRFCONV_NO_ONE_LAUNCH_MLP=1 does the same up front).' % where)




def _env_families(name):
    v = __import__('os').environ.get(name)
    if v is None:
        return False
    v = v.strip().lower()
    return True if v in ('', '1', 'all') else frozenset(q.strip() for q in v.split(',') if q.strip())


class _State:
    no_join = False
    no_fork = False
    no_prefold = False
    no_mask_fold = __import__('os').environ.get('CRFCONV_NO_MASK_FOLD') is not None
    no_combine_fold = _env_families('CRFCONV_NO_COMBINE_FOLD')
    small_mlp_disabled = __import__('os').environ.get('CRFCONV_NO_ONE_LAUNCH_MLP') is not None
    small_bwd_one_launch = __import__('os').environ.get('CRFCONV_SMALL_BWD_TWO_LAUNCHES') is None
    dw_hosts_mats = __import__('os').environ.get('CRFCONV_NO_TAIL_RIDERS') is None
    mfma_min_rows = 12288
    mf_block = __import__('os').environ.get('CRFCONV_MF_BLOCK', 'auto')
    mf_block_min_rows = 65536
    mf_block_min_locality = 0.6


state = _State()
```

### crfconv_amd/ops/defer.py

```python
import ctypes

import torch

from .. import _lib
from ..graph import ptr, stream_ptr
from ._base import state

_DEFER = {'on': False, 'jobs': [], 'partials': [], 'red64': [], 'pc_wide': [], 'tn': [], 'late_calls': [], 'late_mats': [], 'folds': [], 'mlpdw': [], 'armed': False,
          'claimed': set()}


class deferred_weight_grads:

    def __init__(self, enabled=True, sink=None):
        self.enabled = enabled
        self.sink = sink

    def __enter__(self):
        self.prev = _DEFER['on']
        self.prev_sink = _DEFER.get('sink')
        _DEFER['on'] = bool(self.enabled)
        _DEFER['sink'] = self.sink
        if not self.prev:
            _DEFER['jobs'], _DEFER['folds'], _DEFER['mlpdw'], _DEFER['armed'], _DEFER['claimed'] = [], [], [], False, set()
# ... 25 lines not shown
        if dst is not None and dst.dtype == torch.float32 and dst.is_contiguous() and dst.numel() == prm.numel():
            _DEFER['claimed'].add(id(prm))
            return dst.view(shape), True
    return torch.empty(shape, dtype=torch.float32, device=dev), False


def _param_ret(prm, buf, direct):
    if direct:
        prm.grad = buf.view_as(prm)
        return None
    return buf


_WGRAD_BATCH_ROWS = 65536


def _defer_weight_grad(g, x, params, has_bias):
    m, Co = g.shape
    Ci = x.shape[1]
    lib = _lib.load()
    nbytes = lib.crfconv_linear_wgrad_workspace(m, Co, Ci)
    ws = torch.empty(nbytes, dtype=torch.uint8, device=g.device)
    want_b = bool(has_bias and params[1].requires_grad)
    if m <= _WGRAD_BATCH_ROWS:
        g, x = g.contiguous(), x.contiguous()
        _DEFER['partials'].append((_lib.WgradJob(g.data_ptr(), x.data_ptr(), m, Co, Ci, 1 if want_b else 0, ws.data_ptr(), nbytes), (g, x)))
        nblk = lib.crfconv_linear_wgrad_nblk(m, Co, Ci)
    else:
        nb = ctypes.c_int(0)
        _lib.call('crfconv_linear_wgrad_partial', ptr(g), ptr(x), m, Co, Ci, 1 if want_b else 0, ptr(ws), nbytes,
                  ctypes.byref(nb), stream_ptr())
        nblk = nb.value
    _DEFER['jobs'].append((params[0], params[1] if want_b else None, ws, nblk, Co, Ci))
    _arm_flush()


def _defer_tn(A, B, out):
    m, ca = A.shape
    cb = B.shape[1]
    lib = _lib.load()
    nbytes = lib.crfconv_linear_wgrad_workspace(m, ca, cb)
    ws = torch.empty(nbytes, dtype=torch.uint8, device=A.device)
    A, B = A.contiguous(), B.contiguous()
    _DEFER['partials'].append((_lib.WgradJob(A.data_ptr(), B.data_ptr(), m, ca, cb, 0, ws.data_ptr(), nbytes), (A, B)))
    _DEFER['tn'].append((ws, lib.crfconv_linear_wgrad_nblk(m, ca, cb), ca * cb, out))
    _arm_flush()


def _arm_flush():
    if not _DEFER['armed']:
        _DEFER['armed'] = True
        torch.autograd.Variable._execution_engine.queue_callback(_flush_weight_grads)


def _defer_fold1_bwd(job, keep, installs):
    _DEFER['folds'].append((job, keep, installs))
    _arm_flush()


def _mlp_dw_ret(deferred, prm, dW, direct, ws, m, ci, co, coef):
    if not deferred:
        return _param_ret(prm, dW, direct)
    _DEFER['mlpdw'].append((_lib.MlpDwJob(ws.data_ptr(), coef.data_ptr(), dW.data_ptr(), m, ci, co), (ws, coef), (prm, dW, direct)))
    _arm_flush()
    return None

# ... 196 lines not shown
```

### crfconv_amd/ops/dense.py

```python
import ctypes

import torch

from .. import _lib
from ..graph import ptr, require_gpu, stream_ptr
from ._base import _f32c, state



def _mfma_ok(m, ci, co):
    return m >= state.mfma_min_rows and bool(_lib.load().crfconv_linear_forward_supported(ci, co))


def _gemm(A, B, bias=None, addend=None, nk=False):
    M, K = A.shape
    N = B.shape[0] if nk else B.shape[1]
    if M == 0:
        return A.new_empty((0, N))
    if not _lib.load().crfconv_gemm_supported(M, N, K):
        raise _lib.CrfConvError('product %d x %d x %d is outside the tiled kernel\'s range (crfconv_gemm_supported)' % (M, N, K))
    A, B = A.contiguous(), B.contiguous()
    C = torch.empty((M, N), dtype=torch.float32, device=A.device)
    _lib.call('crfconv_gemm', ptr(A), ptr(B), ptr(None if bias is None else bias.contiguous()),
              ptr(None if addend is None else addend.contiguous()), M, N, K, 1 if nk else 0, ptr(C), stream_ptr())
    return C


def _gemm_tn(A, B):
    m, ca = A.shape
    cb = B.shape[1]
    if m == 0:
        return A.new_zeros((ca, cb))
    return _wgrad(A.contiguous(), B.contiguous())[0]


def _wgrad(g, x, has_bias=False, out=None):
    m, co = g.shape
    ci = x.shape[1]
    dW = torch.empty((co, ci), dtype=torch.float32, device=g.device) if out is None else out
    db = torch.empty(co, dtype=torch.float32, device=g.device) if has_bias else None
    nbytes = _lib.load().crfconv_linear_wgrad_workspace(m, co, ci)
    ws = torch.empty(nbytes, dtype=torch.uint8, device=g.device)
    _lib.call('crfconv_linear_wgrad', ptr(g), ptr(x), m, co, ci, ptr(dW), ptr(db), ptr(ws), nbytes, stream_ptr())
    return dW, db


def _weight_grad(g, x, params, has_bias):
    if _defer_ok(params):
        _defer_weight_grad(g, x, params, has_bias)
        return None, None
    return _wgrad(g, x, has_bias)


def _mfma_matmul(x, W, b, transpose_w, want_stats=False):
    m, ci = x.shape
    co = W.shape[1] if transpose_w else W.shape[0]
    y = torch.empty((m, co), dtype=torch.float32, device=x.device)
    rec = None
    if want_stats:
        nrec = _lib.load().crfconv_linear_forward_stat_records(m)
        rec = torch.empty((nrec, 4, co), dtype=torch.float32, device=x.device)
    _lib.call('crfconv_linear_forward', ptr(x), ptr(W), ptr(b), m, ci, co, 1 if transpose_w else 0, ptr(y), ptr(rec),
              stream_ptr())
    return y, rec


class _Linear(torch.autograd.Function):

    @staticmethod
    def forward(ctx, x, W, b, want_stats):
        x = x.contiguous()
        Wc = W.contiguous()
        ctx.save_for_backward(x, Wc)
        ctx.set_materialize_grads(False)
        ctx.has_bias = b is not None
        ctx.params = (W, b)
        m, ci = x.shape
# ... 109 lines not shown
        gx = torch.empty_like(x)
        dgamma = torch.empty(C, dtype=torch.float32, device=x.device)
        dbeta = torch.empty(C, dtype=torch.float32, device=x.device)
        nbytes = _lib.load().crfconv_bn_workspace(m, C)
        ws = torch.empty(nbytes, dtype=torch.uint8, device=x.device)
        _lib.call('crfconv_bn_backward', ptr(gy), ptr(x), ptr(coef), m, C, 1 if ctx.use_batch else 0, float(ctx.slope),
                  ptr(gx), ptr(dgamma), ptr(dbeta), ptr(ws), nbytes, stream_ptr())
        return gx, dgamma, dbeta, None, None, None, None, None, None, None


def bn_act(x, bn, training, slope=1.0, records=None):
    shape = x.shape
    C = shape[-1]
    use_batch = training or bn.running_mean is None
    if training:
        tick(bn)
    mom = 0.1 if bn.momentum is None else bn.momentum
    keep_stats = training or not use_batch
    rm, rv = (bn.running_mean, bn.running_var) if keep_stats else (None, None)
    if C % 4:
        Cp = (C + 3) // 4 * 4
        pad = lambda t, v: None if t is None else torch.nn.functional.pad(t, (0, Cp - C), value=v)
        rmp, rvp = pad(rm, 0.0), pad(rv, 1.0)
        y = _BNAct.apply(pad(x.reshape(-1, C), 0.0), pad(bn.weight, 1.0), pad(bn.bias, 0.0), rmp, rvp, mom, bn.eps, use_batch, slope, None)
        if training and rm is not None:
            with torch.no_grad():
                rm.copy_(rmp[:C])
                rv.copy_(rvp[:C])
        return y[:, :C].reshape(shape)
    y = _BNAct.apply(x.reshape(-1, C), bn.weight, bn.bias, rm, rv, mom, bn.eps, use_batch, slope, records)
    return y.reshape(shape)


from .defer import _defer_ok, _defer_weight_grad
```

### crfconv_amd/ops/mlp.py

```python
import ctypes

import torch

from .. import _lib
from ..graph import ptr, require_gpu, stream_ptr
from ._base import _f32c, _mlp_ticket, _ticket, gridsync_ws, state



class JoinMask:
    __slots__ = ('slope', 'folded')

    def __init__(self):
        self.slope = None
        self.folded = False


def _take_mask(mask, ok):
    if mask is None or mask.slope is None or mask.folded or state.no_mask_fold or not ok:
        return None
    mask.folded = True
    return float(mask.slope)


# ... 316 lines not shown
        g = torch.zeros((table.m_tgt, co), dtype=torch.float32, device=dev) if g is None else _f32c(g)
        rev_ptr, rev_eid = table.reverse
        gA = torch.empty((m, co), dtype=torch.float32, device=dev)
        _lib.call('crfconv_neighbor_maxpool_backward', ptr(g), ptr(arg), ptr(rev_ptr), ptr(rev_eid), table.K, m, co, ptr(gA), stream_ptr())
        return (*_stream_bwd(ctx.prm, x, W, y, coef, gA, 1.0, ctx.needs_input_grad[0], True, g_alias), None, None, None, None, None, None)


def mlp_block_pool(x, W, bn, table, fork=False):
    if state.no_join or table.padded:
        return None
    m, ci = x.shape
    co = W.shape[0]
    if m != table.m_src or not (mlp_block_ok(x, W, None, bn, True) and not _mlp_small_ok(m, ci, co)):
        return None
    require_gpu(x, W)
    tick(bn)
    if _use_fork(fork, x):
        return _MLPBlockPool.apply(x, W, *_bn_args(bn), table, True)
    out = _MLPBlockPool.apply(x, W, *_bn_args(bn), table, False)
    return (out, x) if fork else out

def _small_bwd_jobs(jobs, n, dev, st):
    if state.small_bwd_one_launch and not state.small_mlp_disabled:
        _lib.call('crfconv_mlp_small_backward_jobs_one_launch', ctypes.cast(jobs, ctypes.c_void_p), n, ptr(_ticket(dev)), ptr(gridsync_ws(dev)), st)
    else:
        _lib.call('crfconv_mlp_small_backward_jobs', ctypes.cast(jobs, ctypes.c_void_p), n, ptr(_ticket(dev)), st)


def _mlp_bwd_jobs(blocks):
    jobs = (_lib.MlpBwdJob * len(blocks))()
    for i, (gA, y, coef, W, add, slope, gY, dX, dgamma, dbeta, ws, mask) in enumerate(blocks):
        m, co = y.shape
        mref, mslope = (None, 1.0) if mask is None else (mask[0].data_ptr(), float(mask[1]))
        jobs[i] = _lib.MlpBwdJob(gA.data_ptr(), y.data_ptr(), coef.data_ptr(), W.data_ptr(), None if add is None else add.data_ptr(), m,
                                 W.shape[1], co, 1, float(slope), gY.data_ptr(), dX.data_ptr(), dgamma.data_ptr(), dbeta.data_ptr(),
                                 ws.data_ptr(), ws.numel(), mref, mslope)
    return jobs


def _small_bwd(gA, y, coef, W, addend, slope, dgamma, dbeta, need_dx, mask=None):
    m, co = y.shape
    ci = W.shape[1]
    dev = y.device
    gY = torch.empty_like(y)
    lib = _lib.load()
    if need_dx and lib.crfconv_mlp_small_backward_supported(m, ci, co) == 1:
        dX = torch.empty((m, ci), dtype=torch.float32, device=dev)
        nbytes = lib.crfconv_mlp_small_backward_workspace(m, co)
        ws = torch.empty(nbytes, dtype=torch.uint8, device=dev)
        add = None if addend is None else addend.contiguous()
        jobs = _mlp_bwd_jobs([(gA, y, coef, W, add, slope, gY, dX, dgamma, dbeta, ws, mask)])
        _small_bwd_jobs(jobs, 1, dev, stream_ptr())
        return gY, dX
    if mask is not None:
        raise _lib.CrfConvError('_small_bwd: a folded join mask needs the fused dX product (%d x %d -> %d)' % (m, ci, co))
    nbytes = lib.crfconv_bn_workspace(m, co)
    ws = torch.empty(nbytes, dtype=torch.uint8, device=dev)
    _lib.call('crfconv_bn_backward', ptr(gA), ptr(y), ptr(coef), m, co, 1, float(slope), ptr(gY), ptr(dgamma), ptr(dbeta), ptr(ws),
              nbytes, stream_ptr())
    return gY, (_gemm(gY, W, addend=addend) if need_dx else None)


def _small_fwd(x, Wc, gamma, beta, run_mean, run_var, momentum, eps, slope, skip=None, join_slope=1.0, fold=None):
    m, ci = x.shape
    co = Wc.shape[0]
    dev = x.device
    lib = _lib.load()
    y = torch.empty((m, co), dtype=torch.float32, device=dev)
    out = torch.empty_like(y)
    coef = torch.empty(4 * co, dtype=torch.float32, device=dev)
    g, b = _f32c(gamma), _f32c(beta)
    if not state.small_mlp_disabled and lib.crfconv_mlp_small_supported(m, ci, co) == 1:
        nbytes = lib.crfconv_mlp_small_workspace(m, co)
        ws = torch.empty(nbytes, dtype=torch.uint8, device=dev)
        sync = gridsync_ws(dev)
        if fold is not None:
            _lib.call('crfconv_mlp_small_forward_join_uv', ctypes.byref(fold[0]), ptr(Wc), m, ci, co, ptr(g), ptr(b), ptr(run_mean),
                      ptr(run_var), float(momentum), float(eps), float(slope), ptr(skip), float(join_slope), ptr(y), ptr(out), ptr(coef),
                      ptr(ws), nbytes, ptr(sync), sync.numel() * 4, stream_ptr())
        elif skip is None:
            _lib.call('crfconv_mlp_small_forward', ptr(x), ptr(Wc), m, ci, co, ptr(g), ptr(b), ptr(run_mean), ptr(run_var),
                      float(momentum), float(eps), float(slope), ptr(y), ptr(out), ptr(coef), ptr(ws), nbytes, ptr(sync),
                      sync.numel() * 4, stream_ptr())
        else:
            _lib.call('crfconv_mlp_small_forward_join', ptr(x), ptr(Wc), m, ci, co, ptr(g), ptr(b), ptr(run_mean), ptr(run_var),
                      float(momentum), float(eps), float(slope), ptr(skip), float(join_slope), ptr(y), ptr(out), ptr(coef), ptr(ws),
                      nbytes, ptr(sync), sync.numel() * 4, stream_ptr())
        return y, out, coef
    nrec = lib.crfconv_gemm_stat_records(m)
    rec = torch.empty((nrec, co, 4), dtype=torch.float32, device=dev)
    if fold is not None:
        _lib.call('crfconv_gemm_stats_uv', ctypes.byref(fold[0]), ptr(Wc), m, co, ci, ptr(y), ptr(rec), stream_ptr())
    else:
        _lib.call('crfconv_gemm_stats', ptr(x), ptr(Wc), m, co, ci, ptr(y), ptr(rec), stream_ptr())
    _lib.call('crfconv_bn_apply_from_records', ptr(rec), nrec, ptr(y), m, co, ptr(g), ptr(b), ptr(run_mean), ptr(run_var),
              float(momentum), float(eps), ptr(skip), float(slope if skip is None else join_slope), ptr(coef), ptr(out), stream_ptr())
    return y, out, coef


def _small_tail(ctx, x, W, y, coef, gA, addend, slope, mask=None):
    outs = [_param_out(q, (W.shape[0],), x.device) for q in ctx.prm[1:]]
    gY, dX = _small_bwd(gA, y, coef, W, addend, slope, outs[0][0], outs[1][0], ctx.needs_input_grad[0], mask)
    dW = _weight_grad(gY, x, ctx.params, False)[0]
    return (dX, dW, *(_param_ret(q, o, k) for q, (o, k) in zip(ctx.prm[1:], outs)))


class _MLPSmallJoin(torch.autograd.Function):

    @staticmethod
    def forward(ctx, x, W, gamma, beta, run_mean, run_var, momentum, eps, skip, slope, mask=None, fold=None):
        x, Wc, skip = x.contiguous(), W.contiguous(), skip.contiguous()
        ctx.mask = mask
        y, out, coef = _small_fwd(x, Wc, gamma, beta, run_mean, run_var, momentum, eps, 1.0, skip, slope, fold)
        ctx.prm = (W, gamma, beta)
        ctx.save_for_backward(x, Wc, y, coef, out)
        ctx.slope = float(slope)
        ctx.params = (W, None)
        return out

    @staticmethod
    def backward(ctx, g):
        x, W, y, coef, out = ctx.saved_tensors
        g1 = _join_g1(ctx, g.contiguous(), out)
        gskip = g1 if ctx.needs_input_grad[8] else None
# ... 37 lines not shown

def _mlp_small_ok(m, ci, co):
    if m >= state.mfma_min_rows:
        return False
    lib = _lib.load()
    if not state.small_mlp_disabled and lib.crfconv_mlp_small_supported(m, ci, co) == 1:
        return True
    return ci % 4 == 0 and co % 4 == 0 and lib.crfconv_mlp_small_backward_supported(m, ci, co) == 1


class _MLPSmall(torch.autograd.Function):

    @staticmethod
    def forward(ctx, x_in, W, gamma, beta, run_mean, run_var, momentum, eps, slope, fork=False, mask=None):
        x = x_in.contiguous()
        Wc = W.contiguous()
        ctx.mask_slope = _take_mask(mask, fork and _lib.load().crfconv_mlp_small_backward_supported(x.shape[0], x.shape[1], Wc.shape[0]) == 1)
        y, out, coef = _small_fwd(x, Wc, gamma, beta, run_mean, run_var, momentum, eps, slope)
        ctx.prm = (W, gamma, beta)
        ctx.save_for_backward(x, Wc, y, coef)
        ctx.slope = float(slope)
        ctx.params = (W, None)
        if fork:
            ctx.set_materialize_grads(False)
            return out, x_in
        return out

    @staticmethod
    def backward(ctx, gA, g_alias=None):
        x, W, y, coef = ctx.saved_tensors
        gA = torch.zeros_like(y) if gA is None else gA.contiguous()
        return (*_small_tail(ctx, x, W, y, coef, gA, None if g_alias is None else g_alias.reshape(x.shape), ctx.slope,
                             None if ctx.mask_slope is None else (x, ctx.mask_slope)), None, None, None, None, None, None, None)


class _MLPSmallGroup(torch.autograd.Function):

    NARG = 10

    @staticmethod
    def forward(ctx, shared, mask, *args):
        n = len(args) // _MLPSmallGroup.NARG
        jobs = [args[i * _MLPSmallGroup.NARG:(i + 1) * _MLPSmallGroup.NARG] for i in range(n)]
        lib = _lib.load()
        st = stream_ptr()
        keep, outs, prm, slopes, forks, tmp = [], [], [], [], [], []
        gs = (_lib.GemmStatsJob * n)()
        ba = (_lib.BnApplyJob * n)()
        for i, (x_in, W, gamma, beta, rm, rv, mom, eps, slope, fork) in enumerate(jobs):
            if x_in is None:
                x_in = jobs[0][0]
            x, Wc = x_in.contiguous(), W.contiguous()
            m, ci = x.shape
            co = Wc.shape[0]
            dev = x.device
            y = torch.empty((m, co), dtype=torch.float32, device=dev)
            out = torch.empty_like(y)
            coef = torch.empty(4 * co, dtype=torch.float32, device=dev)
            nrec = lib.crfconv_gemm_stat_records(m)
            rec = torch.empty((nrec, co, 4), dtype=torch.float32, device=dev)
            g, b = _f32c(gamma), _f32c(beta)
            gs[i] = _lib.GemmStatsJob(x.data_ptr(), Wc.data_ptr(), m, co, ci, y.data_ptr(), rec.data_ptr())
            ba[i] = _lib.BnApplyJob(rec.data_ptr(), nrec, y.data_ptr(), m, co, g.data_ptr(), b.data_ptr(),
                                    None if rm is None else rm.data_ptr(), None if rv is None else rv.data_ptr(), float(mom), float(eps),
                                    None, float(slope), coef.data_ptr(), out.data_ptr())
            keep += [x, Wc, y, coef]
# ... 113 lines not shown

class _Cat2(torch.autograd.Function):

    @staticmethod
    def forward(ctx, xa, xb):
        xa, xb = xa.contiguous(), xb.contiguous()
        m, ca = xa.shape
        cb = xb.shape[1]
        out = torch.empty((m, ca + cb), dtype=torch.float32, device=xa.device)
        _lib.call('crfconv_cat2', ptr(xa), ptr(xb), m, ca, cb, ptr(out), stream_ptr())
        ctx.widths = (ca, cb)
        return out

    @staticmethod
    def backward(ctx, g):
        ca, cb = ctx.widths
        g = g.contiguous()
        m = g.shape[0]
        ga = torch.empty((m, ca), dtype=torch.float32, device=g.device)
        gb = torch.empty((m, cb), dtype=torch.float32, device=g.device)
        _lib.call('crfconv_split2', ptr(g), m, ca, cb, ptr(ga), ptr(gb), stream_ptr())
        return ga, gb


def cat2(xa, xb):
    ca, cb = xa.shape[-1], xb.shape[-1]
    if not (xa.is_cuda and xb.is_cuda and xa.dtype == torch.float32 and xb.dtype == torch.float32
            and xa.shape[:-1] == xb.shape[:-1] and ca % 4 == 0 and cb % 4 == 0 and ca >= 4 and cb >= 4 and xa.numel() > 0):
        return torch.cat([xa, xb], dim=-1)
    out = _Cat2.apply(xa.reshape(-1, ca), xb.reshape(-1, cb))
    return out.reshape(xa.shape[:-1] + (ca + cb,))


def mlp_block_cat(xa, xb, W, bn, training, slope=1.0):
    if xa.dim() != xb.dim() or xa.shape[:-1] != xb.shape[:-1]:
        return None
    ca, cb = xa.shape[-1], xb.shape[-1]
    m = xa.numel() // ca
    probe = xa.new_empty((1, ca + cb))
    if not (ca % 4 == 0 and cb % 4 == 0 and xb.dtype == torch.float32 and m >= state.mfma_min_rows
            and mlp_block_ok(probe.expand(m, ca + cb), W, None, bn, training)):
        return None
    require_gpu(xa, xb, W)
    tick(bn)
    out = _MLPBlockCat.apply(xa.reshape(-1, ca), xb.reshape(-1, cb), W, *_bn_args(bn), slope)
    return out.reshape(xa.shape[:-1] + (W.shape[0],))


def mlp_block_ok(x, W, bias, bn, training):
    if not training or bias is not None or x.dtype != torch.float32 or not bn.affine:
        return False
    m = x.numel() // x.shape[-1]
    ci, co = x.shape[-1], W.shape[0]
    if bn.running_mean is None:
        return False
    if _mlp_small_ok(m, ci, co):
        return True
    return (_mfma_ok(m, ci, co) and co % 4 == 0
            and _lib.load().crfconv_mlp_backward_supported(m, ci, co) == 1)


def mlp_block(x, W, bn, slope=1.0, fork=False, input_mask=None):
    require_gpu(x, W)
    shape = x.shape
    tick(bn)
    x2 = x.reshape(-1, shape[-1])
    fn = _MLPSmall if _mlp_small_ok(x2.shape[0], shape[-1], W.shape[0]) else _MLPBlock
    if _use_fork(fork, x2):
        out, alias = fn.apply(x2, W, *_bn_args(bn), slope, True, input_mask)
        return out.reshape(shape[:-1] + (W.shape[0],)), alias.reshape(shape)
    out = fn.apply(x2, W, *_bn_args(bn), slope, False, None)
    out = out.reshape(shape[:-1] + (W.shape[0],))
    return (out, x) if fork else out


def run_lin_bn(seq, x):
    mods = list(seq)
    i = 0
    while i < len(mods):
        lin = mods[i]
        if not isinstance(lin, torch.nn.Linear):
            raise _lib.CrfConvError('run_lin_bn: expected a Linear at position %d, got %s' % (i, type(lin).__name__))
        bn = mods[i + 1] if i + 1 < len(mods) and isinstance(mods[i + 1], torch.nn.BatchNorm1d) else None
        j = i + 1 + (bn is not None)
        act = mods[j] if j < len(mods) and isinstance(mods[j], torch.nn.LeakyReLU) else None
        slope = act.negative_slope if act is not None else 1.0
        co = lin.out_features
        if bn is not None and co % 4 == 0 and co <= 1024 and bn.affine and x.dtype == torch.float32:
            if mlp_block_ok(x, lin.weight, lin.bias, bn, seq.training):
                x = mlp_block(x, lin.weight, bn, slope)
            else:
                records = None
                if seq.training:
                    x, records = linear(x, lin.weight, lin.bias, want_stats=True)
                else:
                    x = linear(x, lin.weight, lin.bias)
                x = bn_act(x, bn, seq.training, slope, records=records)
        else:
            x = linear(x, lin.weight, lin.bias)
            if bn is not None:
                if not bn.affine:
                    raise _lib.CrfConvError('run_lin_bn: affine BatchNorm only (csrc/bn.hip)')
                x = bn_act(x, bn, seq.training, slope)
            elif act is not None:
                x = _LRelu.apply(x, slope)
        i = j + (act is not None)
    return x


from .rows import _LRelu
from .defer import _mlp_param_outs, _mlp_param_rets, _param_out, _param_ret
from .dense import _gemm, _mfma_matmul, _mfma_ok, _weight_grad, bn_act, linear, tick
```

### include/crfconv_amd.h

```cpp
#ifndef CRFCONV_AMD_H
#define CRFCONV_AMD_H

#include <stddef.h>
#include <stdint.h>

#ifdef __cplusplus
extern "C" {
#endif

typedef void* crf_stream_t;

enum {
    CRF_OK = 0,
    CRF_ERR_ARG = -1,
    CRF_ERR_HIP = -2,
    CRF_ERR_UNSUPPORTED = -3,
    CRF_ERR_WORKSPACE = -4
};

#define CRFCONV_ABI_VERSION 1
int crfconv_abi_version(void);
const char* crfconv_last_error(void);


// ... 199 lines not shown
                                       size_t workspace_bytes, unsigned* ticket, crf_stream_t stream);

int crfconv_pointconv_fold1(const float* W1, const float* gamma1, const float* beta1, const double* mom,
                            double n_edges, float* run_mean, float* run_var, float momentum, float eps,
                            int use_batch, int d, float* A1, float* b1, double* aux1, crf_stream_t stream);
int crfconv_pointconv_fold1_bwd(const float* W1, const float* gamma1, const double* mom, const double* aux1,
                                const double* dA1b1, float eps, int use_batch, int d, float* dW1,
                                float* dgamma1, float* dbeta1, const double* dW2_f64, float* dW2_f32, crf_stream_t stream);
typedef struct {
    const float* W1; const float* gamma1; const float* beta1; const double* mom; double n_edges;
    float* run_mean; float* run_var; float momentum; float eps; int32_t use_batch; int32_t d;
    float* A1; float* b1; double* aux1;
} crf_fold1_job;
int crfconv_pointconv_fold1_batched(const crf_fold1_job* jobs, int njobs, crf_stream_t stream);
typedef struct {
    const float* W1; const float* gamma1; const double* mom; const double* aux1; const double* dA1b1;
    float eps; int32_t use_batch; int32_t d; int32_t pad_;
    float* dW1; float* dgamma1; float* dbeta1; const double* dW2_f64; float* dW2_f32;
} crf_fold1_bwd_job;
int crfconv_pointconv_fold1_bwd_batched(const crf_fold1_bwd_job* jobs, int njobs, crf_stream_t stream);
int crfconv_pointconv_fold2(const double* stats, const float* shift, const float* gamma2, const float* beta2,
                            double n_edges, float* run_mean, float* run_var, float momentum, float eps,
                            int use_batch, int d, float* a2, float* b2, double* aux2, crf_stream_t stream);
int crfconv_pointconv_fold2_bwd(const double* red, const float* shift, const double* aux2, const float* gamma2,
                                double n_edges, int use_batch, int d, float* ca, float* cb, float* cc,
                                float* dgamma2, float* dbeta2, crf_stream_t stream);

size_t crfconv_linear_wgrad_workspace(int64_t M, int Co, int Ci);
int crfconv_linear_wgrad(const float* G, const float* X, int64_t M, int Co, int Ci, float* dW, float* db,
                         void* workspace, size_t workspace_bytes, crf_stream_t stream);
typedef struct { const float* partial; float* out; int32_t nblk; int32_t nslots; } crf_reduce_job;
int crfconv_linear_wgrad_partial(const float* G, const float* X, int64_t M, int Co, int Ci, int want_bias,
                                 void* workspace, size_t workspace_bytes, int* nblk_out, crf_stream_t stream);
typedef struct { const float* G; const float* X; int64_t M; int Co; int Ci; int want_bias; void* workspace; size_t workspace_bytes; } crf_wgrad_job;
int crfconv_linear_wgrad_nblk(int64_t M, int Co, int Ci);
int crfconv_linear_wgrad_partial_jobs(const crf_wgrad_job* jobs, int njobs, crf_stream_t stream);
int crfconv_reduce_jobs(const crf_reduce_job* jobs, int njobs, crf_stream_t stream);
int crfconv_reduce_jobs_both(const crf_reduce_job* jobs, int njobs, const crf_reduce64_job* jobs64, int njobs64, crf_stream_t stream);

size_t crfconv_gridsync_workspace(void);
int crfconv_gridsync_fail_word(void);
int crfconv_mlp_small_supported(int64_t M, int Ci, int Co);
size_t crfconv_mlp_small_workspace(int64_t M, int Co);
int crfconv_mlp_small_forward(const float* X, const float* W, int64_t M, int Ci, int Co, const float* gamma,
                              const float* beta, float* run_mean, float* run_var, float momentum, float eps, float slope,
                              float* Y, float* A, float* coef, void* workspace, size_t workspace_bytes, void* sync_ws,
                              size_t sync_bytes, crf_stream_t stream);

int crfconv_mlp_small_forward_join(const float* X, const float* W, int64_t M, int Ci, int Co, const float* gamma,
                                   const float* beta, float* run_mean, float* run_var, float momentum, float eps, float slope,
                                   const float* skip, float join_slope, float* Y, float* A, float* coef, void* workspace,
                                   size_t workspace_bytes, void* sync_ws, size_t sync_bytes, crf_stream_t stream);
int crfconv_mlp_small_forward_uv_supported(int Ci);
int crfconv_mlp_small_forward_join_uv(const crf_uv_fold* f, const float* W, int64_t M, int Ci, int Co, const float* gamma,
                                      const float* beta, float* run_mean, float* run_var, float momentum, float eps, float slope,
                                      const float* skip, float join_slope, float* Y, float* A, float* coef, void* ws, size_t ws_bytes,
                                      void* sync_ws, size_t sync_bytes, crf_stream_t stream);

size_t crfconv_ticket_bytes(void);
int crfconv_mlp_backward_supported(int64_t M, int Ci, int Co);
size_t crfconv_mlp_backward_workspace(int64_t M, int Ci, int Co);
int crfconv_mlp_backward(const float* gA, const float* Y, const float* X, const float* W, const float* coef, float slope,
                         int64_t M, int Ci, int Co, float* dX, float* dW, float* dgamma, float* dbeta, void* workspace,
                         size_t workspace_bytes, unsigned* ticket, crf_stream_t stream);
typedef struct { const void* workspace; const float* coef; float* dW; int64_t M; int32_t Ci; int32_t Co; } crf_mlp_dw_job;
int crfconv_mlp_dw_jobs(const crf_mlp_dw_job* jobs, int njobs, crf_stream_t stream);
int crfconv_mlp_dw_jobs_hosting(const crf_mlp_dw_job* jobs, int njobs, const float* const* c, const float* const* Q,
                                const float* const* gQ, const float* const* gP, const int* H, int n, float* const* dc,
                                crf_stream_t stream);
int crfconv_mlp_backward_add(const float* gA, const float* Y, const float* X, const float* W, const float* coef, float slope,
                             int64_t M, int Ci, int Co, const float* dX_add, float* dX, float* dW, float* dgamma, float* dbeta,
                             void* workspace, size_t workspace_bytes, unsigned* ticket, crf_stream_t stream);
int crfconv_mlp_backward_add_mask(const float* gA, const float* Y, const float* X, const float* W, const float* coef, float slope,
                                  int64_t M, int Ci, int Co, const float* dX_add, float mask_slope, float* dX, float* dW,
                                  float* dgamma, float* dbeta, void* workspace, size_t workspace_bytes, unsigned* ticket,
                                  crf_stream_t stream);
int crfconv_linear_forward_cat(const float* Xa, const float* Xb, int split, const float* W, const float* bias, int64_t M,
                               int Ci, int Co, float* Y, float* stat_rec, crf_stream_t stream);
int crfconv_linear_forward_uv_supported(int Ci, int Co);
int crfconv_linear_forward_uv(const crf_uv_fold* f, const float* W, int64_t M, int Ci, int Co, float* Y, float* stat_rec,
                              crf_stream_t stream);
int crfconv_mlp_backward_cat(const float* gA, const float* Y, const float* Xa, const float* Xb, int split, const float* W,
                             const float* coef, float slope, int64_t M, int Ci, int Co, float* dXa, float* dXb, float* dW,
                             float* dgamma, float* dbeta, void* workspace, size_t workspace_bytes, unsigned* ticket,
                             crf_stream_t stream);

size_t crfconv_bn_workspace(int64_t M, int C);
int crfconv_bn_forward(const float* x, int64_t M, int C, const float* gamma, const float* beta, float* run_mean,
                       float* run_var, float momentum, float eps, int use_batch_stats, float slope, float* coef,
                       float* y, void* workspace, size_t workspace_bytes, crf_stream_t stream);
int crfconv_bn_backward(const float* gy, const float* x, const float* coef, int64_t M, int C, int training,
                        float slope, float* gx, float* dgamma, float* dbeta, void* workspace,
                        size_t workspace_bytes, crf_stream_t stream);

int crfconv_bn_apply(const float* x, int64_t M, int C, const float* coef, float slope, float* y, crf_stream_t stream);

int crfconv_linear_forward_supported(int Ci, int Co);
size_t crfconv_linear_forward_stat_records(int64_t M);
int crfconv_linear_forward(const float* X, const float* W, const float* bias, int64_t M, int Ci, int Co,
                           int transpose_w, float* Y, float* stat_rec, crf_stream_t stream);
int crfconv_cat2(const float* xa, const float* xb, int64_t m, int ca, int cb, float* out, crf_stream_t stream);
int crfconv_split2(const float* g, int64_t m, int ca, int cb, float* ga, float* gb, crf_stream_t stream);
int crfconv_add_i64(int64_t* x, int64_t n, int64_t delta, crf_stream_t stream);
int crfconv_gate_mark(uint64_t* gate, crf_stream_t stream);
int crfconv_gate_wait(uint64_t* gate, int max_wait_us, crf_stream_t stream);

int crfconv_mlp_small_backward_supported(int64_t M, int Ci, int Co);
size_t crfconv_mlp_small_backward_workspace(int64_t M, int Co);
int crfconv_mlp_small_backward(const float* gA, const float* Y, const float* coef, const float* W, const float* addend, int64_t M,
                               int Ci, int Co, int training, float slope, float* gY, float* dX, float* dgamma, float* dbeta,
                               void* workspace, size_t workspace_bytes, unsigned* ticket, crf_stream_t stream);
size_t crfconv_gemm_stat_records(int64_t M);
int crfconv_gemm_stats(const float* A, const float* B, int64_t M, int N, int K, float* C, float* stat_rec, crf_stream_t stream);
int crfconv_gemm_stats_uv_supported(int64_t M, int N, int K);
int crfconv_gemm_stats_uv(const crf_uv_fold* f, const float* B, int64_t M, int N, int K, float* C, float* stat_rec, crf_stream_t stream);
typedef struct { const float* A; const float* B; int64_t M; int N; int K; float* C; float* stat_rec; } crf_gemm_stats_job;
int crfconv_gemm_stats_jobs(const crf_gemm_stats_job* jobs, int njobs, crf_stream_t stream);
typedef struct { const float* stat_rec; int64_t nrec; const float* x; int64_t M; int C; const float* gamma; const float* beta;
                 float* run_mean; float* run_var; float momentum; float eps; const float* skip; float slope; float* coef; float* y;
} crf_bn_apply_job;
int crfconv_bn_apply_from_records_jobs(const crf_bn_apply_job* jobs, int njobs, crf_stream_t stream);
typedef struct { const float* gA; const float* Y; const float* coef; const float* W; const float* addend; int64_t M; int Ci; int Co;
                 int training; float slope; float* gY; float* dX; float* dgamma; float* dbeta; void* workspace; size_t workspace_bytes;
                 const float* mask_ref; float mask_slope;
} crf_mlp_bwd_job;
int crfconv_mlp_small_backward_jobs(const crf_mlp_bwd_job* jobs, int njobs, unsigned* ticket, crf_stream_t stream);
int crfconv_mlp_small_backward_jobs_one_launch(const crf_mlp_bwd_job* jobs, int njobs, unsigned* ticket, unsigned* sync_ws,
                                               crf_stream_t stream);
typedef struct { const float* A; const float* B; float* C; int64_t M; int N; int K; } crf_gemm_job;
int crfconv_gemm_jobs(const crf_gemm_job* jobs, int njobs, crf_stream_t stream);
int crfconv_gemm_supported(int64_t M, int N, int K);
int crfconv_gemm(const float* A, const float* B, const float* bias, const float* addend, int64_t M, int N, int K,
                 int b_is_nk, float* C, crf_stream_t stream);
int crfconv_bn_coef_from_records(const float* stat_rec, int64_t M, int C, const float* gamma, const float* beta,
                                 float* run_mean, float* run_var, float momentum, float eps, float* coef,
                                 crf_stream_t stream);
int crfconv_bn_apply_from_records(const float* stat_rec, int64_t nrec, const float* x, int64_t M, int C, const float* gamma,
                                  const float* beta, float* run_mean, float* run_var, float momentum, float eps, const float* skip,
                                  float slope, float* coef, float* y, crf_stream_t stream);
int crfconv_bn_coef_from_nrecords(const float* stat_rec, int64_t nrec, int64_t M, int C, const float* gamma, const float* beta,
                                  float* run_mean, float* run_var, float momentum, float eps, float* coef, crf_stream_t stream);

int crfconv_spd_inverse(const float* M, int H, float* Q, crf_stream_t stream);
int crfconv_spd_inverse_wide(const float* M, int H, float* Q, crf_stream_t stream);
int crfconv_crf_matrices(const float* c, int H, float* Q, float* P, crf_stream_t stream);
int crfconv_crf_matrices_backward(const float* c, const float* Q, const float* dQ, const float* dP, int H,
                                  float* dc, crf_stream_t stream);
int crfconv_crf_matrices_batched(const float* const* c, const int* H, int n, float* const* Q, float* const* P,
                                 crf_stream_t stream);
int crfconv_crf_matrices_backward_batched(const float* const* c, const float* const* Q, const float* const* gQ,
                                          const float* const* gP, const int* H, int n, float* const* dc,
                                          crf_stream_t stream);

int crfconv_neighbor_maxpool_forward(const float* x, const int32_t* idx32, int K, int64_t m_tgt,
                                     int C, float* out, int32_t* arg, crf_stream_t stream);
int crfconv_neighbor_maxpool_affine_forward(const float* x, const float* coef, const int32_t* idx32, int K, int64_t m_tgt,
                                            int C, float* out, int32_t* arg, crf_stream_t stream);
// ... 167 lines not shown
```

Baseline: 45.58 M points/s.

## Fuse channel concat into small-MLP forward, dX split, and weight-grad kernels

Adds a two-pointer operand path to the small MLP GEMM kernels, so concatenated inputs (xa, xb) are read directly instead of being materialised first. A split output writes dX straight into two separate tensors, and a column-offset weight-grad covers the concatenated input. Small-row cat blocks now go through a new _MLPSmallCat autograd node, where they previously fell back. This is meant to remove concat and split copies and extra launches on low-resolution levels, at the cost of more kernel template variants and a branch per load.

```diff
diff --git a/crfconv_amd/_lib.py b/crfconv_amd/_lib.py
--- a/crfconv_amd/_lib.py
+++ b/crfconv_amd/_lib.py
@@ -74,6 +74,7 @@
     'crfconv_pointconv_fold2_bwd': (_i, [_vp, _vp, _vp, _vp, ctypes.c_double, _i, _i, _vp, _vp, _vp, _vp, _vp, _vp]),
     'crfconv_linear_wgrad_workspace': (_sz, [_i64, _i, _i]),
     'crfconv_linear_wgrad': (_i, [_vp, _vp, _i64, _i, _i, _vp, _vp, _vp, _sz, _vp]),
+    'crfconv_linear_wgrad_cat': (_i, [_vp, _vp, _vp, _i, _i64, _i, _i, _vp, _vp, _sz, _vp]),
     'crfconv_random_subsets': (_i, [_vp, _vp, _vp, _vp, _i, _u64, _vp, _vp]),
     'crfconv_upindex_workspace': (_sz, [_i64, _i64]),
     'crfconv_upindex_from_table': (_i, [_vp, _vp, _vp, _vp, _i64, _i64, _i, _i64, _vp, _vp, _sz, _vp]),
@@ -94,6 +95,9 @@
     'crfconv_linear_forward_uv_supported': (_i, [_i, _i]),
     'crfconv_linear_forward_uv': (_i, [_vp, _vp, _i64, _i, _i, _vp, _vp, _vp]),
     'crfconv_mlp_small_forward_uv_supported': (_i, [_i]),
+    'crfconv_mlp_small_forward_cat': (_i, [_vp, _vp, _i, _vp, _i64, _i, _i, _vp, _vp, _vp, _vp, _f, _f, _f, _vp, _vp, _vp, _vp, _sz, _vp, _sz, _vp]),
+    'crfconv_gemm_stats_cat_supported': (_i, [_i64, _i, _i, _i]),
+    'crfconv_gemm_stats_cat': (_i, [_vp, _vp, _i, _vp, _i64, _i, _i, _vp, _vp, _vp]),
     'crfconv_mlp_small_forward_join_uv': (_i, [_vp, _vp, _i64, _i, _i, _vp, _vp, _vp, _vp, _f, _f, _f, _vp, _f, _vp, _vp, _vp, _vp, _sz, _vp, _sz, _vp]),
     'crfconv_gemm_stats_uv_supported': (_i, [_i64, _i, _i]),
     'crfconv_gemm_stats_uv': (_i, [_vp, _vp, _i64, _i, _i, _vp, _vp, _vp]),
@@ -271,7 +275,7 @@
                 ('M', ctypes.c_int64), ('Ci', ctypes.c_int32), ('Co', ctypes.c_int32), ('training', ctypes.c_int32), ('slope', ctypes.c_float),
                 ('gY', ctypes.c_void_p), ('dX', ctypes.c_void_p), ('dgamma', ctypes.c_void_p), ('dbeta', ctypes.c_void_p),
                 ('workspace', ctypes.c_void_p), ('workspace_bytes', ctypes.c_size_t),
-                ('mask_ref', ctypes.c_void_p), ('mask_slope', ctypes.c_float)]
+                ('mask_ref', ctypes.c_void_p), ('mask_slope', ctypes.c_float), ('dXb', ctypes.c_void_p), ('dx_split', ctypes.c_int32)]
 
 
 class UvFold(ctypes.Structure):
@@ -288,7 +292,8 @@
 
 class WgradJob(ctypes.Structure):
     _fields_ = [('G', ctypes.c_void_p), ('X', ctypes.c_void_p), ('M', ctypes.c_int64), ('Co', ctypes.c_int32), ('Ci', ctypes.c_int32),
-                ('want_bias', ctypes.c_int32), ('workspace', ctypes.c_void_p), ('workspace_bytes', ctypes.c_size_t)]
+                ('want_bias', ctypes.c_int32), ('workspace', ctypes.c_void_p), ('workspace_bytes', ctypes.c_size_t),
+                ('ld_partial', ctypes.c_int32), ('col0', ctypes.c_int32)]
 
 
 class RevJob(ctypes.Structure):
diff --git a/crfconv_amd/csrc/gemm.hip b/crfconv_amd/csrc/gemm.hip
--- a/crfconv_amd/csrc/gemm.hip
+++ b/crfconv_amd/csrc/gemm.hip
@@ -47,6 +47,8 @@
     unsigned* fail = nullptr;
     const float* mref = nullptr;
     float mslope = 1.f;
+    float* C2 = nullptr;
+    int csplit = 0;
 };
 constexpr int GM_PRO_LDS = 6 * GM_PRO_MAXK + 4;
 
@@ -57,15 +59,18 @@
 }
 
 constexpr int GM_UV_MAXK = 128;
-template <int WM, int WN, int WR, int WC, bool BNK, bool VEC, bool PRO, bool STATS, bool UV = false>
+template <int WM, int WN, int WR, int WC, bool BNK, bool VEC, bool PRO, bool STATS, bool UV = false, bool CAT = false, bool CSPLIT = false>
 __device__ __forceinline__ void gemm_tile(const float* __restrict__ A, const float* __restrict__ B,
                                           const float* __restrict__ bias, const float* __restrict__ addend,
                                           int M, int N, int K, float* __restrict__ C, const GemmPro& pro,
                                           float* __restrict__ stat_rec, const unsigned bx, const unsigned by,
                                           float* __restrict__ lds ,
                                           const unsigned gridx = 0 ,
-                                          const UvFold* __restrict__ uv = nullptr, float* __restrict__ uvc = nullptr) {
+                                          const UvFold* __restrict__ uv = nullptr, float* __restrict__ uvc = nullptr,
+                                          const float* __restrict__ A2 = nullptr, const int asplit = 0) {
     static_assert(WR * WC * WAVE == GM_BLOCK, "four wavefronts");
+    static_assert(!CAT || (VEC && !PRO && !UV), "the two-pointer operand: aligned widths, the plain / STATS product");
+    static_assert(!CSPLIT || PRO, "the split result: the dX product");
     static_assert(!UV || (VEC && !PRO), "the combine prologue: aligned widths, not the dX product");
     static_assert(!PRO || (VEC && !BNK), "the prologue form is the dX product of aligned widths");
     constexpr int BM = 16 * WM * WR, BN = 16 * WN * WC;
@@ -94,7 +99,13 @@
             if constexpr (PRO || UV) r.y[i] = zero4;
             if (NA4 % GM_BLOCK != 0 && q >= NA4) continue;
             const int row = m0 + q / (GM_BK / 4), k = kc + 4 * (q % (GM_BK / 4));
-            if (row < M) r.a[i] = gm_ld4<VEC>(A + (int64_t)row * K + k, K - k);
+            if constexpr (CAT) {
+                if (row < M)
+                    r.a[i] = k < asplit ? gm_ld4<VEC>(A + (int64_t)row * asplit + k, asplit - k)
+                                        : gm_ld4<VEC>(A2 + (int64_t)row * (K - asplit) + (k - asplit), K - k);
+            } else {
+                if (row < M) r.a[i] = gm_ld4<VEC>(A + (int64_t)row * K + k, K - k);
+            }
             if constexpr (PRO) {
                 if (row < M) r.y[i] = gm_ld4<VEC>(pro.Y + (int64_t)row * K + k, K - k);
             }
@@ -321,6 +332,9 @@
                 }
             }
             float* cp = C + (int64_t)row * N + n;
+            if constexpr (CSPLIT) {
+                cp = n < pro.csplit ? C + (int64_t)row * pro.csplit + n : pro.C2 + (int64_t)row * (N - pro.csplit) + (n - pro.csplit);
+            }
             if constexpr (VEC) {
                 *reinterpret_cast<float4*>(cp) = o;
             } else {
@@ -414,6 +428,17 @@
     else
         gemm_tile<1, 1, 2, 2, true, true, false, true, true>(U, B, nullptr, nullptr, M, N, K, C, GemmPro(), rec, bx, by, lds, 0, &uv, s_uv);
 }
+__global__ __launch_bounds__(GM_BLOCK) void gemm_stats_cat_kernel(const float* __restrict__ Xa, const float* __restrict__ Xb, const int split,
+                                                                  const float* __restrict__ B, const int M, const int N, const int K,
+                                                                  float* __restrict__ C, float* __restrict__ rec, const int tiles_x, const int wide) {
+    const unsigned tx = (unsigned)tiles_x;
+    const unsigned bx = (unsigned)uni((int)(blockIdx.x % tx)), by = (unsigned)uni((int)(blockIdx.x / tx));
+    __shared__ __attribute__((aligned(16))) float lds[gemm_lds_floats<1, 2, 2, 2, true, false>()];
+    if (wide)
+        gemm_tile<1, 2, 2, 2, true, true, false, true, false, true>(Xa, B, nullptr, nullptr, M, N, K, C, GemmPro(), rec, bx, by, lds, 0, nullptr, nullptr, Xb, split);
+    else
+        gemm_tile<1, 1, 2, 2, true, true, false, true, false, true>(Xa, B, nullptr, nullptr, M, N, K, C, GemmPro(), rec, bx, by, lds, 0, nullptr, nullptr, Xb, split);
+}
 struct GemmProJobs {
     const float* A[GG_MAX]; const float* B[GG_MAX]; const float* addend[GG_MAX]; float* C[GG_MAX];
     GemmPro pro[GG_MAX];
@@ -421,6 +446,7 @@
     int tile_base[GG_MAX + 1];
     int njobs;
 };
+template <bool CSPLIT>
 __global__ __launch_bounds__(GM_BLOCK) void gemm_pro_jobs_kernel(const GemmProJobs t) {
     int j = 0;
     while (j + 1 < t.njobs && t.tile_base[j + 1] <= (int)blockIdx.x) ++j;
@@ -428,14 +454,15 @@
     GemmPro pro;
     pro.Y = uni(t.pro[j].Y); pro.coef = uni(t.pro[j].coef); pro.fin = uni(t.pro[j].fin); pro.slope = uni(t.pro[j].slope); pro.gY = uni(t.pro[j].gY);
     pro.mref = uni(t.pro[j].mref); pro.mslope = uni(t.pro[j].mslope);
+    if constexpr (CSPLIT) { pro.C2 = uni(t.pro[j].C2); pro.csplit = uni(t.pro[j].csplit); }
     const unsigned tx = (unsigned)uni(t.tiles_x[j]);
     const unsigned bx = (unsigned)uni((int)(local % tx)), by = (unsigned)uni((int)(local / tx));
     __shared__ __attribute__((aligned(16))) float lds[gemm_lds_floats<1, 2, 2, 2, false, true>()];
     if (uni(t.wide[j]))
-        gemm_tile<1, 2, 2, 2, false, true, true, false>(uni(t.A[j]), uni(t.B[j]), nullptr, uni(t.addend[j]), uni(t.M[j]), uni(t.N[j]), uni(t.K[j]), uni(t.C[j]),
+        gemm_tile<1, 2, 2, 2, false, true, true, false, false, false, CSPLIT>(uni(t.A[j]), uni(t.B[j]), nullptr, uni(t.addend[j]), uni(t.M[j]), uni(t.N[j]), uni(t.K[j]), uni(t.C[j]),
                                                         pro, nullptr, bx, by, lds, tx);
     else
-        gemm_tile<1, 1, 2, 2, false, true, true, false>(uni(t.A[j]), uni(t.B[j]), nullptr, uni(t.addend[j]), uni(t.M[j]), uni(t.N[j]), uni(t.K[j]), uni(t.C[j]),
+        gemm_tile<1, 1, 2, 2, false, true, true, false, false, false, CSPLIT>(uni(t.A[j]), uni(t.B[j]), nullptr, uni(t.addend[j]), uni(t.M[j]), uni(t.N[j]), uni(t.K[j]), uni(t.C[j]),
                                                         pro, nullptr, bx, by, lds, tx);
 }
 
@@ -572,6 +599,7 @@
 }
 
 struct SmallBwdSync { unsigned* done[GG_MAX]; int nsum; };
+template <bool CSPLIT>
 __global__ __launch_bounds__(GM_BLOCK) void mlp_small_bwd_jobs_kernel(const TileSumJobs ts, const GemmProJobs t, const SmallBwdSync sy) {
     __shared__ __attribute__((aligned(16))) float lds[gemm_lds_floats<1, 2, 2, 2, false, true>()];
     static_assert(sizeof(TileSumLds) <= sizeof(lds), "the tile-sum workgroups use the product's buffer");
@@ -586,14 +614,15 @@
     GemmPro pro;
     pro.Y = uni(t.pro[j].Y); pro.coef = uni(t.pro[j].coef); pro.fin = uni(t.pro[j].fin); pro.slope = uni(t.pro[j].slope); pro.gY = uni(t.pro[j].gY);
     pro.mref = uni(t.pro[j].mref); pro.mslope = uni(t.pro[j].mslope);
+    if constexpr (CSPLIT) { pro.C2 = uni(t.pro[j].C2); pro.csplit = uni(t.pro[j].csplit); }
     pro.sync = uni(t.pro[j].sync); pro.need = (unsigned)uni((int)t.pro[j].need); pro.nprod = (unsigned)uni((int)t.pro[j].nprod); pro.fail = uni(t.pro[j].fail);
     const unsigned tx = (unsigned)uni(t.tiles_x[j]);
     const unsigned bx = (unsigned)uni((int)(local % tx)), by = (unsigned)uni((int)(local / tx));
     if (uni(t.wide[j]))
-        gemm_tile<1, 2, 2, 2, false, true, true, false>(uni(t.A[j]), uni(t.B[j]), nullptr, uni(t.addend[j]), uni(t.M[j]), uni(t.N[j]), uni(t.K[j]), uni(t.C[j]),
+        gemm_tile<1, 2, 2, 2, false, true, true, false, false, false, CSPLIT>(uni(t.A[j]), uni(t.B[j]), nullptr, uni(t.addend[j]), uni(t.M[j]), uni(t.N[j]), uni(t.K[j]), uni(t.C[j]),
                                                         pro, nullptr, bx, by, lds, tx);
     else
-        gemm_tile<1, 1, 2, 2, false, true, true, false>(uni(t.A[j]), uni(t.B[j]), nullptr, uni(t.addend[j]), uni(t.M[j]), uni(t.N[j]), uni(t.K[j]), uni(t.C[j]),
+        gemm_tile<1, 1, 2, 2, false, true, true, false, false, false, CSPLIT>(uni(t.A[j]), uni(t.B[j]), nullptr, uni(t.addend[j]), uni(t.M[j]), uni(t.N[j]), uni(t.K[j]), uni(t.C[j]),
                                                         pro, nullptr, bx, by, lds, tx);
 }
 }
@@ -624,7 +653,7 @@
     crf_mlp_bwd_job job;
     job.gA = gA; job.Y = Y; job.coef = coef; job.W = W; job.addend = addend; job.M = M; job.Ci = Ci; job.Co = Co; job.training = training;
     job.slope = slope; job.gY = gY; job.dX = dX; job.dgamma = dgamma; job.dbeta = dbeta; job.workspace = workspace; job.workspace_bytes = workspace_bytes;
-    job.mask_ref = nullptr; job.mask_slope = 1.f;
+    job.mask_ref = nullptr; job.mask_slope = 1.f; job.dXb = nullptr; job.dx_split = 0;
     return crfconv_mlp_small_backward_jobs(&job, 1, ticket, stream);
 }
 
@@ -644,6 +673,7 @@
     for (int j = 0; j < crf::GG_MAX; ++j) sy.done[j] = nullptr;
     sy.nsum = 0;
     int64_t blocks = 0, tiles = 0;
+    bool split = false;
     for (int j = 0; j <= crf::GG_MAX; ++j) {
         ts.blk_base[j] = (int)blocks;
         gp.tile_base[j] = (int)tiles;
@@ -671,6 +701,10 @@
         crf::GemmPro pro;
         pro.Y = b.Y; pro.coef = b.coef; pro.fin = fin; pro.slope = b.slope; pro.gY = b.gY;
         pro.mref = b.mask_ref; pro.mslope = b.mask_slope;
+        CRF_REQUIRE(b.dXb == nullptr || (b.dx_split > 0 && b.dx_split < b.Ci && b.dx_split % 4 == 0), CRF_ERR_ARG,
+                    "job %d: split dX needs 0 < split < Ci, a multiple of 4 (split=%d Ci=%d)", j, b.dx_split, b.Ci);
+        pro.C2 = b.dXb; pro.csplit = b.dXb != nullptr ? b.dx_split : b.Ci;
+        split = split || b.dXb != nullptr;
         gp.A[j] = b.gA; gp.B[j] = b.W; gp.addend[j] = b.addend; gp.C[j] = b.dX; gp.pro[j] = pro; gp.M[j] = (int)b.M; gp.N[j] = b.Ci; gp.K[j] = b.Co;
         gp.tiles_x[j] = (int)((b.M + 31) / 32);
         gp.wide[j] = crf::gm_wide(b.M, b.Ci) ? 1 : 0;
@@ -691,13 +725,15 @@
     hipStream_t st = crf::as_stream(stream);
     if (sync_ws != nullptr) {
         sy.nsum = (int)blocks;
-        hipLaunchKernelGGL(crf::mlp_small_bwd_jobs_kernel, dim3((unsigned)(blocks + tiles)), dim3(crf::GM_BLOCK), 0, st, ts, gp, sy);
+        if (split) hipLaunchKernelGGL(crf::mlp_small_bwd_jobs_kernel<true>, dim3((unsigned)(blocks + tiles)), dim3(crf::GM_BLOCK), 0, st, ts, gp, sy);
+        else hipLaunchKernelGGL(crf::mlp_small_bwd_jobs_kernel<false>, dim3((unsigned)(blocks + tiles)), dim3(crf::GM_BLOCK), 0, st, ts, gp, sy);
         CRF_LAUNCH_CHECK();
         return CRF_OK;
     }
     hipLaunchKernelGGL(crf::bn_bwd_tile_sums_jobs_kernel, dim3((unsigned)blocks), dim3(256), 0, st, ts);
     CRF_LAUNCH_CHECK();
-    hipLaunchKernelGGL(crf::gemm_pro_jobs_kernel, dim3((unsigned)tiles), dim3(crf::GM_BLOCK), 0, st, gp);
+    if (split) hipLaunchKernelGGL(crf::gemm_pro_jobs_kernel<true>, dim3((unsigned)tiles), dim3(crf::GM_BLOCK), 0, st, gp);
+    else hipLaunchKernelGGL(crf::gemm_pro_jobs_kernel<false>, dim3((unsigned)tiles), dim3(crf::GM_BLOCK), 0, st, gp);
     CRF_LAUNCH_CHECK();
     return CRF_OK;
 }
@@ -751,6 +787,23 @@
     CRF_REQUIRE(tiles < ((int64_t)1 << 31), CRF_ERR_UNSUPPORTED, "too many tiles");
     hipLaunchKernelGGL(crf::gemm_stats_uv_kernel, dim3((unsigned)tiles), dim3(crf::GM_BLOCK), 0, crf::as_stream(stream), f->U, B, (int)M, N, K, C,
                        stat_rec, tiles_x, wide, uv);
+    CRF_LAUNCH_CHECK();
+    return CRF_OK;
+}
+
+extern "C" int crfconv_gemm_stats_cat_supported(int64_t M, int N, int K, int split) {
+    return (M >= 1 && M < ((int64_t)1 << 31) && N >= 4 && K >= 8 && N % 4 == 0 && K % 4 == 0 && split >= 4 && split < K && split % 4 == 0) ? 1 : 0;
+}
+extern "C" int crfconv_gemm_stats_cat(const float* Xa, const float* Xb, int split, const float* B, int64_t M, int N, int K, float* C,
+                                      float* stat_rec, void* stream) {
+    CRF_REQUIRE(Xa && Xb && B && C && stat_rec, CRF_ERR_ARG, "null pointer");
+    CRF_REQUIRE(crfconv_gemm_stats_cat_supported(M, N, K, split), CRF_ERR_UNSUPPORTED,
+                "gemm_stats_cat %lld x %d x %d split %d: N, K, split multiples of 4, 0 < split < K", (long long)M, N, K, split);
+    const int tiles_x = (int)((M + 31) / 32), wide = crf::gm_wide(M, N) ? 1 : 0;
+    const int64_t tiles = (int64_t)tiles_x * ((N + (wide ? 63 : 31)) / (wide ? 64 : 32));
+    CRF_REQUIRE(tiles < ((int64_t)1 << 31), CRF_ERR_UNSUPPORTED, "too many tiles");
+    hipLaunchKernelGGL(crf::gemm_stats_cat_kernel, dim3((unsigned)tiles), dim3(crf::GM_BLOCK), 0, crf::as_stream(stream), Xa, Xb, split, B, (int)M, N,
+                       K, C, stat_rec, tiles_x, wide);
     CRF_LAUNCH_CHECK();
     return CRF_OK;
 }
diff --git a/crfconv_amd/csrc/linear.hip b/crfconv_amd/csrc/linear.hip
--- a/crfconv_amd/csrc/linear.hip
+++ b/crfconv_amd/csrc/linear.hip
@@ -17,7 +17,7 @@
                                                          float* __restrict__ partial_b ) {
     __shared__ float s_red[WG_RED_BUFS * TCO * TCI * 256];
     __shared__ float s_b[WG_WAVES * TCO * 16];
-    wgrad_body<TCO, TCI>(G, X, M, Co, Ci, rows_per_block, partial, partial_b, blockIdx.x, blockIdx.y, blockIdx.z, s_red, s_b);
+    wgrad_body<TCO, TCI>(G, X, M, Co, Ci, rows_per_block, partial, partial_b, blockIdx.x, blockIdx.y, blockIdx.z, s_red, s_b, Ci, 0);
 }
 
 __global__ __launch_bounds__(WG_BLOCK) void wgrad_jobs_any_kernel(const WgJobTable t) {
@@ -434,7 +434,10 @@
         CRF_REQUIRE(jb.M > 0 && jb.M < ((int64_t)1 << 31) && jb.Co > 0 && jb.Ci > 0 && jb.Co <= 4096 && jb.Ci <= 4096, CRF_ERR_ARG,
                     "job %d: bad shape M=%lld Co=%d Ci=%d", j, (long long)jb.M, jb.Co, jb.Ci);
         CRF_REQUIRE((reinterpret_cast<uintptr_t>(jb.workspace) & 255) == 0, CRF_ERR_ARG, "job %d: workspace must be 256-byte aligned", j);
-        CRF_REQUIRE(jb.workspace_bytes >= crfconv_linear_wgrad_workspace(jb.M, jb.Co, jb.Ci), CRF_ERR_WORKSPACE, "job %d: workspace too small", j);
+        CRF_REQUIRE(jb.ld_partial == 0 || (!jb.want_bias && jb.col0 >= 0 && jb.col0 + jb.Ci <= jb.ld_partial && jb.ld_partial <= 4096), CRF_ERR_ARG,
+                    "job %d: column block %d + %d of %d (no bias)", j, jb.col0, jb.Ci, jb.ld_partial);
+        CRF_REQUIRE(jb.workspace_bytes >= crfconv_linear_wgrad_workspace(jb.M, jb.Co, jb.ld_partial > 0 ? jb.ld_partial : jb.Ci), CRF_ERR_WORKSPACE,
+                    "job %d: workspace too small", j);
     }
     for (int j0 = 0; j0 < njobs; j0 += WJ_MAX) {
         WgJobTable t;
@@ -537,6 +540,31 @@
                            Co, db);
         CRF_LAUNCH_CHECK();
     }
+    return CRF_OK;
+}
+
+extern "C" int crfconv_linear_wgrad_cat(const float* G, const float* Xa, const float* Xb, int ca, int64_t M, int Co, int Ci, float* dW,
+                                        void* workspace, size_t workspace_bytes, crf_stream_t stream) {
+    CRF_REQUIRE(G && Xa && Xb && dW && workspace, CRF_ERR_ARG, "null pointer");
+    CRF_REQUIRE(M > 0 && M < ((int64_t)1 << 31) && Co > 0 && Ci > 1 && Co <= 4096 && Ci <= 4096 && ca > 0 && ca < Ci, CRF_ERR_ARG,
+                "bad shape M=%lld Co=%d Ci=%d split=%d", (long long)M, Co, Ci, ca);
+    CRF_REQUIRE(workspace_bytes >= crfconv_linear_wgrad_workspace(M, Co, Ci), CRF_ERR_WORKSPACE, "workspace too small");
+    void* aligned = reinterpret_cast<void*>((reinterpret_cast<uintptr_t>(workspace) + 255) & ~(uintptr_t)255);
+    crf_wgrad_job jobs[2];
+    jobs[0].G = G; jobs[0].X = Xa; jobs[0].M = M; jobs[0].Co = Co; jobs[0].Ci = ca; jobs[0].want_bias = 0; jobs[0].workspace = aligned;
+    jobs[0].workspace_bytes = workspace_bytes; jobs[0].ld_partial = Ci; jobs[0].col0 = 0;
+    jobs[1] = jobs[0];
+    jobs[1].X = Xb; jobs[1].Ci = Ci - ca; jobs[1].col0 = ca;
+    WgJobTable t;
+    int64_t blocks = 0;
+    wg_fill_table(jobs, 2, t, blocks);
+    CRF_REQUIRE(blocks < ((int64_t)1 << 31), CRF_ERR_UNSUPPORTED, "too many workgroups");
+    hipStream_t st = as_stream(stream);
+    hipLaunchKernelGGL(wgrad_jobs_any_kernel, dim3((unsigned)blocks), dim3(WG_BLOCK), 0, st, t);
+    CRF_LAUNCH_CHECK();
+    hipLaunchKernelGGL(wgrad_reduce_kernel, dim3((unsigned)cdiv((int64_t)Co * Ci, 64)), dim3(256), 0, st, reinterpret_cast<const float*>(aligned),
+                       t.nblk[0], Co * Ci, dW);
+    CRF_LAUNCH_CHECK();
     return CRF_OK;
 }
 
diff --git a/crfconv_amd/csrc/mlp_small.hip b/crfconv_amd/csrc/mlp_small.hip
--- a/crfconv_amd/csrc/mlp_small.hip
+++ b/crfconv_amd/csrc/mlp_small.hip
@@ -16,7 +16,7 @@
 #endif
 
 constexpr int SM_UV_MAXK = 128;
-template <int TCO, bool UV>
+template <int TCO, bool UV, bool CAT = false>
 __device__ __forceinline__ void mlp_small_fwd_body(const float* __restrict__ X, const float* __restrict__ W,
                                                    int M, int Ci, int Co, const float* __restrict__ gamma,
                                                    const float* __restrict__ beta, float* __restrict__ run_mean,
@@ -24,7 +24,9 @@
                                                    float slope, float* __restrict__ Y, float* __restrict__ A,
                                                    float* __restrict__ coef, float* __restrict__ rec,
                                                    unsigned* __restrict__ sync_ws,
-                                                   const float* __restrict__ skip, float join_slope, const UvFold& uv) {
+                                                   const float* __restrict__ skip, float join_slope, const UvFold& uv,
+                                                   const float* __restrict__ Xb = nullptr, const int xsplit = 0) {
+    static_assert(!(UV && CAT), "one operand form per kernel");
     __shared__ float sWbuf[2][SM_COLS * SM_LD];
     __shared__ __attribute__((aligned(16))) float s_uv[UV ? 2 : 1][UV ? SM_UV_MAXK : 4];
     __shared__ double s_comb[2][SM_BLOCK];
@@ -37,7 +39,12 @@
     const int rb = blockIdx.x, co_base = blockIdx.y * COLS;
     const int r = rb * SM_ROWS + wave * 16 + rr;
     const bool rv = r < M;
-    const float* xrow = X + (int64_t)(rv ? r : 0) * Ci;
+    const float* xrow = X + (int64_t)(rv ? r : 0) * (CAT ? xsplit : Ci);
+    [[maybe_unused]] const float* xbrow = CAT ? Xb + (int64_t)(rv ? r : 0) * (Ci - xsplit) : nullptr;
+    auto ldx = [&](int k0) -> float4 {
+        if constexpr (CAT) return k0 < xsplit ? ld4(xrow + k0) : ld4(xbrow + (k0 - xsplit));
+        else return ld4(xrow + k0);
+    };
     const float4 zero4 = make_float4(0.f, 0.f, 0.f, 0.f);
     [[maybe_unused]] const float* vrow = UV ? uv.V + (int64_t)(rv ? r : 0) * Ci : nullptr;
     if constexpr (UV) {
@@ -70,7 +77,7 @@
 #pragma unroll
     for (int c = 0; c < 4; ++c) {
         const int k0 = 16 * c + 4 * g;
-        xv[c] = (rv && k0 < Ci) ? ld4(xrow + k0) : zero4;
+        xv[c] = (rv && k0 < Ci) ? ldx(k0) : zero4;
         if constexpr (UV) vn[c] = (rv && k0 < Ci) ? ld4(vrow + k0) : zero4;
     }
 #pragma unroll
@@ -90,7 +97,7 @@
 #pragma unroll
             for (int c = 0; c < 4; ++c) {
                 const int k0 = kn + 16 * c + 4 * g;
-                xn[c] = (rv && k0 < Ci) ? ld4(xrow + k0) : zero4;
+                xn[c] = (rv && k0 < Ci) ? ldx(k0) : zero4;
                 if constexpr (UV) vn[c] = (rv && k0 < Ci) ? ld4(vrow + k0) : zero4;
             }
         }
@@ -277,6 +284,18 @@
                                   join_slope, uv);
 }
 
+template <int TCO>
+__global__ __launch_bounds__(SM_BLOCK) void mlp_small_fwd_cat_kernel(const float* __restrict__ Xa, const float* __restrict__ Xb, const int xsplit,
+                                                                     const float* __restrict__ W, int M, int Ci, int Co,
+                                                                     const float* __restrict__ gamma, const float* __restrict__ beta,
+                                                                     float* __restrict__ run_mean, float* __restrict__ run_var, float momentum,
+                                                                     float eps, float slope, float* __restrict__ Y, float* __restrict__ A,
+                                                                     float* __restrict__ coef, float* __restrict__ rec,
+                                                                     unsigned* __restrict__ sync_ws) {
+    mlp_small_fwd_body<TCO, false, true>(Xa, W, M, Ci, Co, gamma, beta, run_mean, run_var, momentum, eps, slope, Y, A, coef, rec, sync_ws,
+                                         nullptr, 1.f, UvFold(), Xb, xsplit);
+}
+
 static int mlp_small_capacity() {
     static int cap = -1;
     if (cap < 0) {
@@ -287,6 +306,8 @@
         if (hipOccupancyMaxActiveBlocksPerMultiprocessor(&per_cu, mlp_small_fwd_kernel<4>, SM_BLOCK, 0) != hipSuccess) return 0;
         if (hipOccupancyMaxActiveBlocksPerMultiprocessor(&per_cu_uv, mlp_small_fwd_uv_kernel<4>, SM_BLOCK, 0) != hipSuccess) return 0;
         if (per_cu_uv < per_cu) per_cu = per_cu_uv;
+        if (hipOccupancyMaxActiveBlocksPerMultiprocessor(&per_cu_uv, mlp_small_fwd_cat_kernel<4>, SM_BLOCK, 0) != hipSuccess) return 0;
+        if (per_cu_uv < per_cu) per_cu = per_cu_uv;
         if (per_cu > 2) per_cu = 2;
         cap = cus * per_cu;
     }
@@ -328,7 +349,8 @@
 static int mlp_small_forward_impl(const float* X, const float* W, int64_t M, int Ci, int Co, const float* gamma,
                                   const float* beta, float* run_mean, float* run_var, float momentum, float eps,
                                   float slope, const float* skip, float join_slope, float* Y, float* A, float* coef, void* ws,
-                                  size_t ws_bytes, void* sync_ws, size_t sync_bytes, crf_stream_t stream, const UvFold* uv = nullptr) {
+                                  size_t ws_bytes, void* sync_ws, size_t sync_bytes, crf_stream_t stream, const UvFold* uv = nullptr,
+                                  const float* Xb = nullptr, int xsplit = 0) {
     CRF_REQUIRE(X && W && gamma && beta && Y && A && coef && ws && sync_ws, CRF_ERR_ARG, "null pointer");
     CRF_REQUIRE(mlp_small_shape_ok(M, Ci, Co), CRF_ERR_UNSUPPORTED, "shape m=%lld Ci=%d Co=%d outside the one-launch kernel",
                 (long long)M, Ci, Co);
@@ -345,13 +367,21 @@
 #define SMU(T) hipLaunchKernelGGL(mlp_small_fwd_uv_kernel<T>, grid, dim3(SM_BLOCK), 0, as_stream(stream), X, W, (int)M, Ci, Co, gamma, beta, \
                                   run_mean, run_var, momentum, eps, slope, Y, A, coef, reinterpret_cast<float*>(ws),                  \
                                   reinterpret_cast<unsigned*>(sync_ws), skip, join_slope, *uv)
-    if (uv != nullptr) {
+#define SMC(T) hipLaunchKernelGGL(mlp_small_fwd_cat_kernel<T>, grid, dim3(SM_BLOCK), 0, as_stream(stream), X, Xb, xsplit, W, (int)M, Ci, Co, gamma, \
+                                  beta, run_mean, run_var, momentum, eps, slope, Y, A, coef, reinterpret_cast<float*>(ws),                    \
+                                  reinterpret_cast<unsigned*>(sync_ws))
+    if (Xb != nullptr) {
+        if (tco == 4) SMC(4);
+        else if (tco == 2) SMC(2);
+        else SMC(1);
+    } else if (uv != nullptr) {
         if (tco == 4) SMU(4);
         else if (tco == 2) SMU(2);
         else SMU(1);
     } else if (tco == 4) SMF(4);
     else if (tco == 2) SMF(2);
     else SMF(1);
+#undef SMC
 #undef SMU
 #undef SMF
     CRF_LAUNCH_CHECK();
@@ -388,3 +418,14 @@
     return mlp_small_forward_impl(f->U, W, M, Ci, Co, gamma, beta, run_mean, run_var, momentum, eps, slope, skip, join_slope, Y, A, coef,
                                   ws, ws_bytes, sync_ws, sync_bytes, stream, &uv);
 }
+
+extern "C" int crfconv_mlp_small_forward_cat(const float* Xa, const float* Xb, int split, const float* W, int64_t M, int Ci, int Co,
+                                             const float* gamma, const float* beta, float* run_mean, float* run_var, float momentum, float eps,
+                                             float slope, float* Y, float* A, float* coef, void* ws, size_t ws_bytes, void* sync_ws,
+                                             size_t sync_bytes, crf_stream_t stream) {
+    CRF_REQUIRE(Xb, CRF_ERR_ARG, "null pointer");
+    CRF_REQUIRE(split >= 4 && split < Ci && split % 4 == 0, CRF_ERR_ARG, "two-operand form needs 0 < split < Ci, a multiple of 4 (split=%d Ci=%d)",
+                split, Ci);
+    return mlp_small_forward_impl(Xa, W, M, Ci, Co, gamma, beta, run_mean, run_var, momentum, eps, slope, nullptr, 1.f, Y, A, coef, ws, ws_bytes,
+                                  sync_ws, sync_bytes, stream, nullptr, Xb, split);
+}
diff --git a/crfconv_amd/csrc/wgrad_body.hpp b/crfconv_amd/csrc/wgrad_body.hpp
--- a/crfconv_amd/csrc/wgrad_body.hpp
+++ b/crfconv_amd/csrc/wgrad_body.hpp
@@ -16,7 +16,8 @@
 __device__ __forceinline__ void wgrad_body(const float* __restrict__ G, const float* __restrict__ X, int64_t M, int Co, int Ci,
                                            int rows_per_block, float* __restrict__ partial ,
                                            float* __restrict__ partial_b , int bx, int by, int bz,
-                                           float* __restrict__ s_red_ , float* __restrict__ s_b_ ) {
+                                           float* __restrict__ s_red_ , float* __restrict__ s_b_ ,
+                                           const int ldp, const int col0) {
     const int lane = threadIdx.x & 63, wave = threadIdx.x >> 6;
     const int co_base = by * 16 * TCO, ci_base = bz * 16 * TCI;
     const int kk = lane >> 4, cc = lane & 15;
@@ -116,7 +117,7 @@
         const int t = threadIdx.x + WG_BLOCK * i;
         const int tile = t >> 8, a = tile / TCI, b = tile % TCI, r = (t >> 4) & 15, j = t & 15;
         const int co = co_base + 16 * a + r, ci = ci_base + 16 * b + j;
-        if (co < Co && ci < Ci) partial[(pb * Co + co) * Ci + ci] = v[i];
+        if (co < Co && ci < Ci) partial[(pb * Co + co) * ldp + col0 + ci] = v[i];
     }
     if (partial_b != nullptr && bz == 0) {
         for (int t = threadIdx.x; t < TCO * 16; t += WG_BLOCK) {
@@ -135,7 +136,7 @@
     const float* X[WJ_MAX];
     float* partial[WJ_MAX];
     float* partial_b[WJ_MAX];
-    int M[WJ_MAX], Co[WJ_MAX], Ci[WJ_MAX], rows_per_block[WJ_MAX], nblk[WJ_MAX], gy[WJ_MAX];
+    int M[WJ_MAX], Co[WJ_MAX], Ci[WJ_MAX], rows_per_block[WJ_MAX], nblk[WJ_MAX], gy[WJ_MAX], ldp[WJ_MAX], col0[WJ_MAX];
     int blk_base[WJ_MAX + 1];
     int njobs;
     unsigned char cls[WJ_MAX];
@@ -149,7 +150,7 @@
     const int local = blk - t.blk_base[lo];
     const int bx = local % t.nblk[lo], rest = local / t.nblk[lo];
     const int by = rest % t.gy[lo], bz = rest / t.gy[lo];
-#define WB(TA, TB) wgrad_body<TA, TB>(t.G[lo], t.X[lo], t.M[lo], t.Co[lo], t.Ci[lo], t.rows_per_block[lo], t.partial[lo], t.partial_b[lo], bx, by, bz, s_red, s_b)
+#define WB(TA, TB) wgrad_body<TA, TB>(t.G[lo], t.X[lo], t.M[lo], t.Co[lo], t.Ci[lo], t.rows_per_block[lo], t.partial[lo], t.partial_b[lo], bx, by, bz, s_red, s_b, t.ldp[lo], t.col0[lo])
     switch (t.cls[lo]) {
         case 44: WB(4, 4); break;
         case 22: WB(2, 2); break;
@@ -201,11 +202,17 @@
     blocks = 0;
     for (int k = 0; k < n; ++k) {
         const crf_wgrad_job& jb = jobs[k];
-        const WgPlan p = wg_plan(jb.M, jb.Co, jb.Ci);
+        WgPlan p = wg_plan(jb.M, jb.Co, jb.Ci);
+        if (jb.ld_partial > 0) {
+            const WgPlan wide = wg_plan(jb.M, jb.Co, jb.ld_partial);
+            p.rows_per_block = wide.rows_per_block;
+            p.nblk = wide.nblk;
+        }
         float* partial = reinterpret_cast<float*>(jb.workspace);
         t.G[k] = jb.G; t.X[k] = jb.X; t.partial[k] = partial;
         t.partial_b[k] = jb.want_bias ? partial + (size_t)p.nblk * jb.Co * jb.Ci : nullptr;
         t.M[k] = (int)jb.M; t.Co[k] = jb.Co; t.Ci[k] = jb.Ci; t.rows_per_block[k] = p.rows_per_block; t.nblk[k] = p.nblk; t.gy[k] = p.gy;
+        t.ldp[k] = jb.ld_partial > 0 ? jb.ld_partial : jb.Ci; t.col0[k] = jb.ld_partial > 0 ? jb.col0 : 0;
         t.cls[k] = (unsigned char)(10 * p.tco + p.tci);
         t.blk_base[k] = (int)blocks;
         blocks += (int64_t)p.nblk * p.gy * p.gz;
@@ -213,7 +220,7 @@
     for (int k = n; k <= WJ_MAX; ++k) t.blk_base[k] = (int)blocks;
     for (int k = n; k < WJ_MAX; ++k) {
         t.G[k] = nullptr; t.X[k] = nullptr; t.partial[k] = nullptr; t.partial_b[k] = nullptr;
-        t.M[k] = 0; t.Co[k] = 1; t.Ci[k] = 1; t.rows_per_block[k] = 64; t.nblk[k] = 1; t.gy[k] = 1; t.cls[k] = 11;
+        t.M[k] = 0; t.Co[k] = 1; t.Ci[k] = 1; t.rows_per_block[k] = 64; t.nblk[k] = 1; t.gy[k] = 1; t.ldp[k] = 1; t.col0[k] = 0; t.cls[k] = 11;
     }
     t.njobs = n;
 }
diff --git a/crfconv_amd/ops/_base.py b/crfconv_amd/ops/_base.py
--- a/crfconv_amd/ops/_base.py
+++ b/crfconv_amd/ops/_base.py
@@ -140,6 +140,7 @@
     no_prefold = False
     no_mask_fold = __import__('os').environ.get('CRFCONV_NO_MASK_FOLD') is not None
     no_combine_fold = _env_families('CRFCONV_NO_COMBINE_FOLD')
+    no_ksplit = _env_families('CRFCONV_NO_KSPLIT')
     small_mlp_disabled = __import__('os').environ.get('CRFCONV_NO_ONE_LAUNCH_MLP') is not None
     small_bwd_one_launch = __import__('os').environ.get('CRFCONV_SMALL_BWD_TWO_LAUNCHES') is None
     dw_hosts_mats = __import__('os').environ.get('CRFCONV_NO_TAIL_RIDERS') is None
diff --git a/crfconv_amd/ops/defer.py b/crfconv_amd/ops/defer.py
--- a/crfconv_amd/ops/defer.py
+++ b/crfconv_amd/ops/defer.py
@@ -81,6 +81,20 @@
                   ctypes.byref(nb), stream_ptr())
         nblk = nb.value
     _DEFER['jobs'].append((params[0], params[1] if want_b else None, ws, nblk, Co, Ci))
+    _arm_flush()
+
+
+def _defer_weight_grad_cat(g, xa, xb, params):
+    m, Co = g.shape
+    ca, cb = xa.shape[1], xb.shape[1]
+    Ci = ca + cb
+    lib = _lib.load()
+    nbytes = lib.crfconv_linear_wgrad_workspace(m, Co, Ci)
+    ws = torch.empty(nbytes, dtype=torch.uint8, device=g.device)
+    g, xa, xb = g.contiguous(), xa.contiguous(), xb.contiguous()
+    for x, c, col0 in ((xa, ca, 0), (xb, cb, ca)):
+        _DEFER['partials'].append((_lib.WgradJob(g.data_ptr(), x.data_ptr(), m, Co, c, 0, ws.data_ptr(), nbytes, Ci, col0), (g, x, ws)))
+    _DEFER['jobs'].append((params[0], None, ws, lib.crfconv_linear_wgrad_nblk(m, Co, Ci), Co, Ci))
     _arm_flush()
 
 
diff --git a/crfconv_amd/ops/dense.py b/crfconv_amd/ops/dense.py
--- a/crfconv_amd/ops/dense.py
+++ b/crfconv_amd/ops/dense.py
@@ -43,6 +43,20 @@
     ws = torch.empty(nbytes, dtype=torch.uint8, device=g.device)
     _lib.call('crfconv_linear_wgrad', ptr(g), ptr(x), m, co, ci, ptr(dW), ptr(db), ptr(ws), nbytes, stream_ptr())
     return dW, db
+
+
+def _weight_grad_cat(g, xa, xb, params):
+    if _defer_ok(params):
+        _defer_weight_grad_cat(g, xa, xb, params)
+        return None
+    m, co = g.shape
+    ca, ci = xa.shape[1], xa.shape[1] + xb.shape[1]
+    dW = torch.empty((co, ci), dtype=torch.float32, device=g.device)
+    nbytes = _lib.load().crfconv_linear_wgrad_workspace(m, co, ci)
+    ws = torch.empty(nbytes, dtype=torch.uint8, device=g.device)
+    _lib.call('crfconv_linear_wgrad_cat', ptr(g.contiguous()), ptr(xa.contiguous()), ptr(xb.contiguous()), ca, m, co, ci, ptr(dW), ptr(ws), nbytes,
+              stream_ptr())
+    return dW
 
 
 def _weight_grad(g, x, params, has_bias):
@@ -218,4 +232,4 @@
     return y.reshape(shape)
 
 
-from .defer import _defer_ok, _defer_weight_grad
+from .defer import _defer_ok, _defer_weight_grad, _defer_weight_grad_cat
diff --git a/crfconv_amd/ops/mlp.py b/crfconv_amd/ops/mlp.py
--- a/crfconv_amd/ops/mlp.py
+++ b/crfconv_amd/ops/mlp.py
@@ -372,20 +372,24 @@
     for i, (gA, y, coef, W, add, slope, gY, dX, dgamma, dbeta, ws, mask) in enumerate(blocks):
         m, co = y.shape
         mref, mslope = (None, 1.0) if mask is None else (mask[0].data_ptr(), float(mask[1]))
+        dXa, dXb, split = (dX[0], dX[1].data_ptr(), dX[0].shape[1]) if isinstance(dX, tuple) else (dX, None, 0)
         jobs[i] = _lib.MlpBwdJob(gA.data_ptr(), y.data_ptr(), coef.data_ptr(), W.data_ptr(), None if add is None else add.data_ptr(), m,
-                                 W.shape[1], co, 1, float(slope), gY.data_ptr(), dX.data_ptr(), dgamma.data_ptr(), dbeta.data_ptr(),
-                                 ws.data_ptr(), ws.numel(), mref, mslope)
+                                 W.shape[1], co, 1, float(slope), gY.data_ptr(), dXa.data_ptr(), dgamma.data_ptr(), dbeta.data_ptr(),
+                                 ws.data_ptr(), ws.numel(), mref, mslope, dXb, split)
     return jobs
 
 
-def _small_bwd(gA, y, coef, W, addend, slope, dgamma, dbeta, need_dx, mask=None):
+def _small_bwd(gA, y, coef, W, addend, slope, dgamma, dbeta, need_dx, mask=None, split=None):
     m, co = y.shape
     ci = W.shape[1]
     dev = y.device
     gY = torch.empty_like(y)
     lib = _lib.load()
     if need_dx and lib.crfconv_mlp_small_backward_supported(m, ci, co) == 1:
-        dX = torch.empty((m, ci), dtype=torch.float32, device=dev)
+        if split is None:
+            dX = torch.empty((m, ci), dtype=torch.float32, device=dev)
+        else:
+            dX = (torch.empty((m, split), dtype=torch.float32, device=dev), torch.empty((m, ci - split), dtype=torch.float32, device=dev))
         nbytes = lib.crfconv_mlp_small_backward_workspace(m, co)
         ws = torch.empty(nbytes, dtype=torch.uint8, device=dev)
         add = None if addend is None else addend.contiguous()
@@ -394,6 +398,8 @@
         return gY, dX
     if mask is not None:
         raise _lib.CrfConvError('_small_bwd: a folded join mask needs the fused dX product (%d x %d -> %d)' % (m, ci, co))
+    if split is not None and need_dx:
+        raise _lib.CrfConvError('_small_bwd: a split input gradient needs the fused dX product (%d x %d -> %d)' % (m, ci, co))
     nbytes = lib.crfconv_bn_workspace(m, co)
     ws = torch.empty(nbytes, dtype=torch.uint8, device=dev)
     _lib.call('crfconv_bn_backward', ptr(gA), ptr(y), ptr(coef), m, co, 1, float(slope), ptr(gY), ptr(dgamma), ptr(dbeta), ptr(ws),
@@ -402,7 +408,13 @@
 
 
 def _small_fwd(x, Wc, gamma, beta, run_mean, run_var, momentum, eps, slope, skip=None, join_slope=1.0, fold=None):
+    xb = None
+    if isinstance(x, tuple):
+        x, xb = x
     m, ci = x.shape
+    split = ci
+    if xb is not None:
+        ci += xb.shape[1]
     co = Wc.shape[0]
     dev = x.device
     lib = _lib.load()
@@ -414,7 +426,11 @@
         nbytes = lib.crfconv_mlp_small_workspace(m, co)
         ws = torch.empty(nbytes, dtype=torch.uint8, device=dev)
         sync = gridsync_ws(dev)
-        if fold is not None:
+        if xb is not None:
+            _lib.call('crfconv_mlp_small_forward_cat', ptr(x), ptr(xb), split, ptr(Wc), m, ci, co, ptr(g), ptr(b), ptr(run_mean), ptr(run_var),
+                      float(momentum), float(eps), float(slope), ptr(y), ptr(out), ptr(coef), ptr(ws), nbytes, ptr(sync), sync.numel() * 4,
+                      stream_ptr())
+        elif fold is not None:
             _lib.call('crfconv_mlp_small_forward_join_uv', ctypes.byref(fold[0]), ptr(Wc), m, ci, co, ptr(g), ptr(b), ptr(run_mean),
                       ptr(run_var), float(momentum), float(eps), float(slope), ptr(skip), float(join_slope), ptr(y), ptr(out), ptr(coef),
                       ptr(ws), nbytes, ptr(sync), sync.numel() * 4, stream_ptr())
@@ -429,7 +445,9 @@
         return y, out, coef
     nrec = lib.crfconv_gemm_stat_records(m)
     rec = torch.empty((nrec, co, 4), dtype=torch.float32, device=dev)
-    if fold is not None:
+    if xb is not None:
+        _lib.call('crfconv_gemm_stats_cat', ptr(x), ptr(xb), split, ptr(Wc), m, co, ci, ptr(y), ptr(rec), stream_ptr())
+    elif fold is not None:
         _lib.call('crfconv_gemm_stats_uv', ctypes.byref(fold[0]), ptr(Wc), m, co, ci, ptr(y), ptr(rec), stream_ptr())
     else:
         _lib.call('crfconv_gemm_stats', ptr(x), ptr(Wc), m, co, ci, ptr(y), ptr(rec), stream_ptr())
@@ -533,6 +551,29 @@
         gA = torch.zeros_like(y) if gA is None else gA.contiguous()
         return (*_small_tail(ctx, x, W, y, coef, gA, None if g_alias is None else g_alias.reshape(x.shape), ctx.slope,
                              None if ctx.mask_slope is None else (x, ctx.mask_slope)), None, None, None, None, None, None, None)
+
+
+class _MLPSmallCat(torch.autograd.Function):
+
+    @staticmethod
+    def forward(ctx, xa, xb, W, gamma, beta, run_mean, run_var, momentum, eps, slope):
+        xa, xb, Wc = xa.contiguous(), xb.contiguous(), W.contiguous()
+        y, out, coef = _small_fwd((xa, xb), Wc, gamma, beta, run_mean, run_var, momentum, eps, slope)
+        ctx.prm = (W, gamma, beta)
+        ctx.save_for_backward(xa, xb, Wc, y, coef)
+        ctx.slope = float(slope)
+        return out
+
+    @staticmethod
+    def backward(ctx, gA):
+        xa, xb, W, y, coef = ctx.saved_tensors
+        want_a, want_b = ctx.needs_input_grad[:2]
+        outs = [_param_out(q, (W.shape[0],), y.device) for q in ctx.prm[1:]]
+        gY, dX = _small_bwd(gA.contiguous(), y, coef, W, None, ctx.slope, outs[0][0], outs[1][0], want_a or want_b, None, xa.shape[1])
+        dxa, dxb = (None, None) if dX is None else dX
+        dW = _weight_grad_cat(gY, xa, xb, (ctx.prm[0], None))
+        return (dxa if want_a else None, dxb if want_b else None, dW, *(_param_ret(q, o, k) for q, (o, k) in zip(ctx.prm[1:], outs)),
+                None, None, None, None, None)
 
 
 class _MLPSmallGroup(torch.autograd.Function):
@@ -712,18 +753,34 @@
     return out.reshape(xa.shape[:-1] + (ca + cb,))
 
 
+def _mlp_small_cat_ok(m, ca, cb, co):
+    ci = ca + cb
+    lib = _lib.load()
+    if not (_mlp_small_ok(m, ci, co) and lib.crfconv_mlp_small_backward_supported(m, ci, co) == 1):
+        return False
+    if not state.small_mlp_disabled and lib.crfconv_mlp_small_supported(m, ci, co) == 1:
+        return True
+    return lib.crfconv_gemm_stats_cat_supported(m, co, ci, ca) == 1
+
+
 def mlp_block_cat(xa, xb, W, bn, training, slope=1.0):
     if xa.dim() != xb.dim() or xa.shape[:-1] != xb.shape[:-1]:
         return None
     ca, cb = xa.shape[-1], xb.shape[-1]
-    m = xa.numel() // ca
+    m = xa.numel() // max(ca, 1)
     probe = xa.new_empty((1, ca + cb))
-    if not (ca % 4 == 0 and cb % 4 == 0 and xb.dtype == torch.float32 and m >= state.mfma_min_rows
+    if not (ca % 4 == 0 and cb % 4 == 0 and ca >= 4 and cb >= 4 and m >= 1 and xb.dtype == torch.float32
             and mlp_block_ok(probe.expand(m, ca + cb), W, None, bn, training)):
         return None
+    node = _MLPBlockCat
+    if m < state.mfma_min_rows:
+        off = state.no_ksplit
+        if off is True or (bool(off) and 'cat' in off) or not _mlp_small_cat_ok(m, ca, cb, W.shape[0]):
+            return None
+        node = _MLPSmallCat
     require_gpu(xa, xb, W)
     tick(bn)
-    out = _MLPBlockCat.apply(xa.reshape(-1, ca), xb.reshape(-1, cb), W, *_bn_args(bn), slope)
+    out = node.apply(xa.reshape(-1, ca), xb.reshape(-1, cb), W, *_bn_args(bn), slope)
     return out.reshape(xa.shape[:-1] + (W.shape[0],))
 
 
@@ -790,4 +847,4 @@
 
 from .rows import _LRelu
 from .defer import _mlp_param_outs, _mlp_param_rets, _param_out, _param_ret
-from .dense import _gemm, _mfma_matmul, _mfma_ok, _weight_grad, bn_act, linear, tick
+from .dense import _gemm, _mfma_matmul, _mfma_ok, _weight_grad, _weight_grad_cat, bn_act, linear, tick
diff --git a/include/crfconv_amd.h b/include/crfconv_amd.h
--- a/include/crfconv_amd.h
+++ b/include/crfconv_amd.h
@@ -255,9 +255,13 @@
 typedef struct { const float* partial; float* out; int32_t nblk; int32_t nslots; } crf_reduce_job;
 int crfconv_linear_wgrad_partial(const float* G, const float* X, int64_t M, int Co, int Ci, int want_bias,
                                  void* workspace, size_t workspace_bytes, int* nblk_out, crf_stream_t stream);
-typedef struct { const float* G; const float* X; int64_t M; int Co; int Ci; int want_bias; void* workspace; size_t workspace_bytes; } crf_wgrad_job;
+typedef struct { const float* G; const float* X; int64_t M; int Co; int Ci; int want_bias; void* workspace; size_t workspace_bytes;
+                 int ld_partial; int col0;
+} crf_wgrad_job;
 int crfconv_linear_wgrad_nblk(int64_t M, int Co, int Ci);
 int crfconv_linear_wgrad_partial_jobs(const crf_wgrad_job* jobs, int njobs, crf_stream_t stream);
+int crfconv_linear_wgrad_cat(const float* G, const float* Xa, const float* Xb, int ca, int64_t M, int Co, int Ci, float* dW,
+                             void* workspace, size_t workspace_bytes, crf_stream_t stream);
 int crfconv_reduce_jobs(const crf_reduce_job* jobs, int njobs, crf_stream_t stream);
 int crfconv_reduce_jobs_both(const crf_reduce_job* jobs, int njobs, const crf_reduce64_job* jobs64, int njobs64, crf_stream_t stream);
 
@@ -274,6 +278,9 @@
                                    const float* beta, float* run_mean, float* run_var, float momentum, float eps, float slope,
                                    const float* skip, float join_slope, float* Y, float* A, float* coef, void* workspace,
                                    size_t workspace_bytes, void* sync_ws, size_t sync_bytes, crf_stream_t stream);
+int crfconv_mlp_small_forward_cat(const float* Xa, const float* Xb, int split, const float* W, int64_t M, int Ci, int Co, const float* gamma,
+                                  const float* beta, float* run_mean, float* run_var, float momentum, float eps, float slope, float* Y,
+                                  float* A, float* coef, void* ws, size_t ws_bytes, void* sync_ws, size_t sync_bytes, crf_stream_t stream);
 int crfconv_mlp_small_forward_uv_supported(int Ci);
 int crfconv_mlp_small_forward_join_uv(const crf_uv_fold* f, const float* W, int64_t M, int Ci, int Co, const float* gamma,
                                       const float* beta, float* run_mean, float* run_var, float momentum, float eps, float slope,
@@ -335,6 +342,9 @@
                                void* workspace, size_t workspace_bytes, unsigned* ticket, crf_stream_t stream);
 size_t crfconv_gemm_stat_records(int64_t M);
 int crfconv_gemm_stats(const float* A, const float* B, int64_t M, int N, int K, float* C, float* stat_rec, crf_stream_t stream);
+int crfconv_gemm_stats_cat_supported(int64_t M, int N, int K, int split);
+int crfconv_gemm_stats_cat(const float* Xa, const float* Xb, int split, const float* B, int64_t M, int N, int K, float* C, float* stat_rec,
+                           crf_stream_t stream);
 int crfconv_gemm_stats_uv_supported(int64_t M, int N, int K);
 int crfconv_gemm_stats_uv(const crf_uv_fold* f, const float* B, int64_t M, int N, int K, float* C, float* stat_rec, crf_stream_t stream);
 typedef struct { const float* A; const float* B; int64_t M; int N; int K; float* C; float* stat_rec; } crf_gemm_stats_job;
@@ -346,6 +356,7 @@
 typedef struct { const float* gA; const float* Y; const float* coef; const float* W; const float* addend; int64_t M; int Ci; int Co;
                  int training; float slope; float* gY; float* dX; float* dgamma; float* dbeta; void* workspace; size_t workspace_bytes;
                  const float* mask_ref; float mask_slope;
+                 float* dXb; int dx_split;
 } crf_mlp_bwd_job;
 int crfconv_mlp_small_backward_jobs(const crf_mlp_bwd_job* jobs, int njobs, unsigned* ticket, crf_stream_t stream);
 int crfconv_mlp_small_backward_jobs_one_launch(const crf_mlp_bwd_job* jobs, int njobs, unsigned* ticket, unsigned* sync_ws,
```

After: 45.81 M points/s, median of 6. Within noise of the previous version (+0.5%).
